# eragonruan/text-detection-ctpn

Hardware: NVIDIA H100
Metric: images/sec @600x900 (higher is better)
Workload: dtype fp32-faithful: fp16 operands + e4m3 cross terms (1 fp16 + 1 e4m3 wgmma per 16 MACs: 2 bf16-rate units per MAC), fp32 accumulate; matmuls around the BiLSTM on bf16x2

## Files before the change

text-detection-ctpn_b200/csrc/common.cuh:

```cuda
#pragma once
#include <cuda_runtime.h>
#include <cuda_bf16.h>
#include <cuda_fp16.h>
#include <stdint.h>
#include <stdio.h>
#include <string.h>

#include "../../include/ctpn_b200.h"

namespace ctpn {

void set_error(const char *fmt, ...);
int cuda_fail(cudaError_t e, const char *what, const char *file, int line);
int current_sm_count(int *sms);

#define CTPN_CUDA(call)                                                        \
  do {                                                                         \
    cudaError_t _e = (call);                                                   \
    if (_e != cudaSuccess) return ::ctpn::cuda_fail(_e, #call, __FILE__, __LINE__); \
  } while (0)

#define CTPN_REQUIRE(cond, ...)                \
  do {                                         \
    if (!(cond)) {                             \
      ::ctpn::set_error(__VA_ARGS__);          \
      return CTPN_ERR_INVALID;                 \
    }                                          \
  } while (0)

#define CTPN_LAUNCH_CHECK()                                                    \
  do {                                                                         \
    cudaError_t _e = cudaGetLastError();                                       \
    if (_e != cudaSuccess) return ::ctpn::cuda_fail(_e, "kernel launch", __FILE__, __LINE__); \
  } while (0)

bool prof_enabled();
struct ProfScope {
  ProfScope(const char *label, double work, cudaStream_t st);
  ~ProfScope();
  cudaStream_t st_;
  int idx_;
};

int conv1_1_tc_ragged(const void *src, int src_is_f32, const float *lut, const float *w_hwio, const float *bias, void *out_planes,
                      int B, int H, int W, int planes, bool outq, float out_s, float out_t, const int *sizes, void *stream);
struct QuantScales { float inv_main, inv_cross, out_s, out_t; };
int conv_tc_run(const void *in_planes, const void *w_planes, const float *bias, void *out, int B, int H, int W, int cin,
                int cout, int taps, int planes, int flags, const QuantScales *q, const int *ext, int ext_shift, void *stream);
int bilstm_ragged(const float *xproj, const float *wh_fw, const float *wh_bw, void *out_planes, int R, int W, int planes,
                  const int *sizes, int rows_per_image, void *stream);

static inline size_t align_up(size_t v, size_t a) { return (v + a - 1) / a * a; }
static inline int ceil_div(int a, int b) { return (a + b - 1) / b; }

__device__ __forceinline__ void split_planes(float a, int planes, __nv_bfloat16 *p) {
  __nv_bfloat16 h0 = __float2bfloat16_rn(a);
  p[0] = h0;
  if (planes > 1) {
    float r1 = __fsub_rn(a, __bfloat162float(h0));
    __nv_bfloat16 h1 = __float2bfloat16_rn(r1);
    p[1] = h1;
    if (planes > 2) {
      float r2 = __fsub_rn(r1, __bfloat162float(h1));
      p[2] = __float2bfloat16_rn(r2);
    }
  }
}

template <int P>
__device__ __forceinline__ void split_planes2(float a, float b, uint32_t (&w)[P]) {
#pragma unroll
  for (int pl = 0; pl < P; ++pl) {
    uint32_t pk;
    asm("cvt.rn.bf16x2.f32 %0, %1, %2;" : "=r"(pk) : "f"(b), "f"(a));
    w[pl] = pk;
    if (pl + 1 < P) {
      a = __fsub_rn(a, __uint_as_float(pk << 16));
      b = __fsub_rn(b, __uint_as_float(pk & 0xffff0000u));
    }
  }
}

constexpr float kResidualGain = 2048.0f;

__device__ __forceinline__ uint32_t f16x2_split(float a, float b, float &ra, float &rb) {
  uint32_t pk;
  asm("cvt.rn.satfinite.f16x2.f32 %0, %1, %2;" : "=r"(pk) : "f"(b), "f"(a));
  const __half2 h = *reinterpret_cast<const __half2 *>(&pk);
  ra = __fsub_rn(a, __low2float(h));
  rb = __fsub_rn(b, __high2float(h));
  return pk;
}
__device__ __forceinline__ uint32_t e4m3x4(float a, float b, float c, float d) {
  uint16_t lo, hi;
  asm("cvt.rn.satfinite.e4m3x2.f32 %0, %1, %2;" : "=h"(lo) : "f"(b), "f"(a));
  asm("cvt.rn.satfinite.e4m3x2.f32 %0, %1, %2;" : "=h"(hi) : "f"(d), "f"(c));
  return (uint32_t)lo | ((uint32_t)hi << 16);
}

__device__ __forceinline__ float2 fmul2_rn(float2 a, float2 b) { return make_float2(__fmul_rn(a.x, b.x), __fmul_rn(a.y, b.y)); }
__device__ __forceinline__ float2 ffma2_rn(float2 a, float2 b, float2 c) {
  return make_float2(__fmaf_rn(a.x, b.x, c.x), __fmaf_rn(a.y, b.y, c.y));
}

__device__ __forceinline__ void f16f8_quad(float v0, float v1, float v2, float v3, float s, float t, float rs, uint32_t &h01,
                                           uint32_t &h23, uint32_t &qv, uint32_t &qr) {
  const float2 a = make_float2(v0, v1), b = make_float2(v2, v3);
  float2 as = a, bs = b;
  if (s != 1.f) {
    as = fmul2_rn(a, make_float2(s, s));
    bs = fmul2_rn(b, make_float2(s, s));
  }
  float2 ra, rb;
  h01 = f16x2_split(as.x, as.y, ra.x, ra.y);
  h23 = f16x2_split(bs.x, bs.y, rb.x, rb.y);
  const float2 at = fmul2_rn(a, make_float2(t, t)), bt = fmul2_rn(b, make_float2(t, t));
  qv = e4m3x4(at.x, at.y, bt.x, bt.y);
  ra = fmul2_rn(ra, make_float2(rs, rs));
  rb = fmul2_rn(rb, make_float2(rs, rs));
  qr = e4m3x4(ra.x, ra.y, rb.x, rb.y);
}

__device__ __forceinline__ uint32_t pack_bf16x2(__nv_bfloat16 lo, __nv_bfloat16 hi) {
  return (uint32_t)__bfloat16_as_ushort(lo) | ((uint32_t)__bfloat16_as_ushort(hi) << 16);
}

__device__ __forceinline__ float bf16_bits_to_float(uint32_t bits16) {
  return __uint_as_float(bits16 << 16);
}

}
```

text-detection-ctpn_b200/csrc/conv1_tc.cu:

```cuda
#include <mutex>

#include "common.cuh"
#include "tc_ptx.cuh"

namespace ctpn {

#ifdef CTPN_DEBUG
#define C1_DBG(p, bit) (((p).debug & (bit)) != 0)
#else
#define C1_DBG(p, bit) false
#endif


constexpr int kC1tThreads = 512;
constexpr int kC1tTileBytes = 128 * 128;
constexpr int kC1tPatch = 3 * 18 * 40;

struct Conv1TcParams {
  const void *src;
  const float *lut, *w, *bias;
  __nv_bfloat16 *out;
  int B, H, W, src_is_f32;
  int tiles_x, tiles_y, total_tiles;
  int debug;
  long long plane_stride;
  float out_s, out_t, out_rs;
  const int *sizes;
};

__device__ __forceinline__ void c1_extent(const Conv1TcParams &p, int b, int &eh, int &ew) {
  eh = p.H; ew = p.W;
  if (p.sizes) {
    eh = min(eh, __ldg(p.sizes + 2 * b));
    ew = min(ew, __ldg(p.sizes + 2 * b + 1));
  }
}

template <int P, int OUTQ>
__global__ void __launch_bounds__(kC1tThreads, 1)
conv1_tc_kernel(const Conv1TcParams p) {
  using namespace ptx;
  extern __shared__ uint8_t smem_raw[];
  const uint32_t raw = smem_u32(smem_raw);
  constexpr int kSPG = P <= 2 ? 2 : 1;
  constexpr int kStages = 2 * kSPG;
  const uint32_t a0 = (raw + 1023u) & ~1023u;
  const uint32_t b0 = a0 + (uint32_t)kStages * P * kC1tTileBytes;
  uint8_t *base = smem_raw + (a0 - raw);
  uint8_t *bsm = base + kStages * P * kC1tTileBytes;
  float *patch = reinterpret_cast<float *>(bsm + P * 64 * 128);
  float *lut_s = patch + 4 * kC1tPatch;
  float *epi = lut_s + 768;
  uint64_t *bars = reinterpret_cast<uint64_t *>(epi + 2 * 128 * 32);
  const uint32_t fullA = smem_u32(bars), emptyA = fullA + 32;

  const int warp = __shfl_sync(0xffffffffu, (int)(threadIdx.x >> 5), 0), lane = threadIdx.x & 31;
  if (threadIdx.x == 0) {
    for (int i = 0; i < 4; ++i) {
      mbar_init(fullA + 8 * i, 128);
      mbar_init(emptyA + 8 * i, 2);
    }
    fence_mbar_init();
  }
  if (!p.src_is_f32)
    for (int i = threadIdx.x; i < 768; i += kC1tThreads) lut_s[i] = p.lut[i];
  for (int i = threadIdx.x; i < 64 * 4; i += kC1tThreads) {
    const int co = i >> 2, chunk = i & 3;
    uint32_t pk[3][4];
#pragma unroll
    for (int j = 0; j < 4; ++j) {
      float v[2];
#pragma unroll
      for (int e = 0; e < 2; ++e) {
        const int k = chunk * 8 + j * 2 + e;
        v[e] = k < 27 ? p.w[k * 64 + co] : (k == 27 ? p.bias[co] : 0.f);
      }
      uint32_t t[P];
      split_planes2<P>(v[0], v[1], t);
#pragma unroll
      for (int pl = 0; pl < P; ++pl) pk[pl][j] = t[pl];
    }
#pragma unroll
    for (int pl = 0; pl < P; ++pl)
      *reinterpret_cast<uint4 *>(bsm + pl * 64 * 128 + co * 128 + ((chunk ^ (co & 7)) << 4)) = make_uint4(pk[pl][0], pk[pl][1], pk[pl][2], pk[pl][3]);
  }
  fence_proxy_async();
  __syncthreads();
  const int tiles_per_img = p.tiles_x * p.tiles_y;

  if (warp < 8) {
    const int grp = warp >> 2;
    const int m = (warp & 3) * 32 + lane, th = m >> 3, tw = m & 7;
    const unsigned tpi = (unsigned)tiles_per_img, tx = (unsigned)p.tiles_x;
    uint32_t raw[2][3];
    unsigned valid = 0;
    auto fetch = [&](int tile) {
      valid = 0;
      if (tile >= p.total_tiles) return;
      const unsigned b = (unsigned)tile / tpi, r = (unsigned)tile % tpi;
      const int y0 = (int)(r / tx) * 16, x0 = (int)(r % tx) * 8;
      int eh, ew;
      c1_extent(p, (int)b, eh, ew);
#pragma unroll
      for (int u = 0; u < 2; ++u) {
        const int i = m + u * 128;
        const int xx = i % 10, yy = i / 10;
        const int gx = x0 + xx - 1, gy = y0 + yy - 1;
        if (i < 180 && gx >= 0 && gx < ew && gy >= 0 && gy < eh && !C1_DBG(p, 1)) {
          const size_t off = (((size_t)b * p.H + gy) * p.W + gx) * 3;
          if (p.src_is_f32) {
            const float *q = reinterpret_cast<const float *>(p.src) + off;
            raw[u][0] = __float_as_uint(q[0]); raw[u][1] = __float_as_uint(q[1]); raw[u][2] = __float_as_uint(q[2]);
          } else {
            const uint8_t *q = reinterpret_cast<const uint8_t *>(p.src) + off;
            raw[u][0] = q[0]; raw[u][1] = q[1]; raw[u][2] = q[2];
          }
          valid |= 1u << u;
        }
      }
    };
    fetch(blockIdx.x + grp * gridDim.x);
    int n = 0;
    for (int tile = blockIdx.x + grp * gridDim.x; tile < p.total_tiles; tile += 2 * gridDim.x, ++n) {
      const int s = grp * kSPG + n % kSPG;
      const uint32_t ph = (uint32_t)(n / kSPG) & 1u;
      float *pt = patch + (grp * 2 + (n & 1)) * kC1tPatch;
#pragma unroll
      for (int u = 0; u < 2; ++u) {
        const int i = m + u * 128;
        if (i < 180) {
          const int xx = i % 10, yy = i / 10;
          float v0 = 0.f, v1 = 0.f, v2 = 0.f;
          if ((valid >> u) & 1u) {
            if (p.src_is_f32) {
              v0 = __uint_as_float(raw[u][0]); v1 = __uint_as_float(raw[u][1]); v2 = __uint_as_float(raw[u][2]);
            } else {
              v0 = lut_s[raw[u][0] * 3 + 0]; v1 = lut_s[raw[u][1] * 3 + 1]; v2 = lut_s[raw[u][2] * 3 + 2];
            }
          }
          pt[(0 * 18 + yy) * 40 + xx] = v0;
          pt[(1 * 18 + yy) * 40 + xx] = v1;
          pt[(2 * 18 + yy) * 40 + xx] = v2;
        }
      }
      fetch(tile + 2 * gridDim.x);
      mbar_wait(emptyA + 8 * s, ph ^ 1u);
      if (grp == 0) asm volatile("bar.sync 1, 128;" ::: "memory");
      else asm volatile("bar.sync 2, 128;" ::: "memory");
      uint8_t *arow = base + s * P * kC1tTileBytes + m * 128;
#pragma unroll
      for (int chunk = 0; chunk < (C1_DBG(p, 2) ? 0 : 4); ++chunk) {
        uint32_t pk[3][4];
#pragma unroll
        for (int j = 0; j < 4; ++j) {
          float v[2];
#pragma unroll
          for (int e = 0; e < 2; ++e) {
            const int k = chunk * 8 + j * 2 + e;
            v[e] = k < 27 ? pt[((k % 3) * 18 + th + k / 9) * 40 + tw + (k / 3) % 3] : (k == 27 ? 1.f : 0.f);
          }
          uint32_t t[P];
          split_planes2<P>(v[0], v[1], t);
#pragma unroll
          for (int pl = 0; pl < P; ++pl) pk[pl][j] = t[pl];
        }
#pragma unroll
        for (int pl = 0; pl < P; ++pl)
          *reinterpret_cast<uint4 *>(arow + pl * kC1tTileBytes + ((chunk ^ (m & 7)) << 4)) = make_uint4(pk[pl][0], pk[pl][1], pk[pl][2], pk[pl][3]);
      }
      fence_proxy_async();
      mbar_arrive(fullA + 8 * s);
    }
  } else {
    const int wg = (warp >> 2) - 2;
    const int cw = warp - 8, chunk = cw >> 2, quarter = cw & 3;
    const int m = quarter * 32 + lane, th = m >> 3, tw = m & 7;
    const int frow = wg * 64 + (warp & 3) * 16 + (lane >> 2);
    constexpr uint32_t kHi = gmma_desc_hi(1024);
    const uint32_t b_lo = gmma_desc_lo(b0);
    float accm[32], accc[32];
    uint4 *stage_w = reinterpret_cast<uint4 *>(epi + chunk * 4096 + quarter * 1024);
    int n = 0;
    for (int tile = blockIdx.x; tile < p.total_tiles; tile += gridDim.x, ++n) {
      const int s = (n & 1) * kSPG + (n >> 1) % kSPG;
      const uint32_t ph = (uint32_t)((n >> 1) / kSPG) & 1u;
      const unsigned b = (unsigned)tile / (unsigned)tiles_per_img, r = (unsigned)tile % (unsigned)tiles_per_img;
      const int y = (int)(r / (unsigned)p.tiles_x) * 16 + th, x = (int)(r % (unsigned)p.tiles_x) * 8 + tw;
      const bool ok = y < p.H && x < p.W;
      int eh, ew;
      c1_extent(p, (int)b, eh, ew);
      const bool live = y < eh && x < ew;
      const long long pix = ((long long)b * p.H + y) * p.W + x;
      const unsigned okmask = __ballot_sync(0xffffffffu, ok);
      long long spix[4];
#pragma unroll
      for (int it = 0; it < 4; ++it) {
        const long long hi = __shfl_sync(0xffffffffu, (int)(pix >> 32), it * 8 + (lane >> 2));
        const unsigned lo = __shfl_sync(0xffffffffu, (unsigned)(pix & 0xffffffffll), it * 8 + (lane >> 2));
        spix[it] = (hi << 32) | lo;
      }
      mbar_wait(fullA + 8 * s, ph);
      const uint32_t a_lo = gmma_desc_lo(a0 + s * P * kC1tTileBytes + wg * 64 * 128);
      wgmma_fence();
#pragma unroll
      for (int i = 0; i < P; ++i)
#pragma unroll
        for (int j = 0; j < P - i; ++j)
#pragma unroll
          for (int k = 0; k < 2; ++k) {
            const uint64_t da = ((uint64_t)kHi << 32) | (a_lo + i * (kC1tTileBytes >> 4) + 2u * k);
            const uint64_t db = ((uint64_t)kHi << 32) | (b_lo + j * ((64 * 128) >> 4) + 2u * k);
            if (i + j == 0) wgmma_bf16(accm, da, db, (uint32_t)k);
            else wgmma_bf16(accc, da, db, (k == 0 && i == 0 && j == 1) ? 0u : 1u);
          }
      wgmma_commit();
      wgmma_wait<0>();
      wgmma_fence_regs(accm);
      if (P > 1) wgmma_fence_regs(accc);
      if ((threadIdx.x & 127) == 0) mbar_arrive(emptyA + 8 * s);
      if (P > 1) {
#pragma unroll
        for (int i = 0; i < 32; ++i) accm[i] = accm[i] + accc[i];
      }
      named_sync(3, 256);
#pragma unroll
      for (int j = 0; j < 8; ++j) {
        const int q = 2 * (j & 3) + ((lane & 3) >> 1);
#pragma unroll
        for (int h = 0; h < 2; ++h) {
          const int row = frow + 8 * h;
          *reinterpret_cast<float2 *>(epi + (j >> 2) * 4096 + row * 32 + ((q ^ (row & 7)) << 2) + 2 * (lane & 1)) =
              make_float2(accm[4 * j + 2 * h], accm[4 * j + 2 * h + 1]);
        }
      }
      named_sync(3, 256);
      if (!C1_DBG(p, 8)) {
        float v[32];
#pragma unroll
        for (int q = 0; q < 8; ++q) {
          const float4 t = *reinterpret_cast<const float4 *>(epi + chunk * 4096 + m * 32 + ((q ^ (m & 7)) << 2));
          v[4 * q + 0] = t.x; v[4 * q + 1] = t.y; v[4 * q + 2] = t.z; v[4 * q + 3] = t.w;
        }
        if (!live) {
#pragma unroll
          for (int i = 0; i < 32; ++i) v[i] = 0.f;
        }
        if (OUTQ) {
          uint32_t wh[16], wq[16];
#pragma unroll
          for (int i = 0; i < 8; ++i) {
            const float v0 = fmaxf(v[4 * i], 0.f), v1 = fmaxf(v[4 * i + 1], 0.f), v2 = fmaxf(v[4 * i + 2], 0.f), v3 = fmaxf(v[4 * i + 3], 0.f);
            f16f8_quad(v0, v1, v2, v3, p.out_s, p.out_t, p.out_rs, wh[2 * i], wh[2 * i + 1], wq[i], wq[8 + i]);
          }
#pragma unroll
          for (int pl = 0; pl < 2; ++pl) {
            __syncwarp();
#pragma unroll
            for (int q = 0; q < 4; ++q) {
              const uint4 val = pl == 0 ? make_uint4(wh[4 * q], wh[4 * q + 1], wh[4 * q + 2], wh[4 * q + 3])
                                        : make_uint4(wq[4 * q], wq[4 * q + 1], wq[4 * q + 2], wq[4 * q + 3]);
              stage_w[lane * 4 + (q ^ ((lane >> 1) & 3))] = val;
            }
            __syncwarp();
            uint8_t *obase = reinterpret_cast<uint8_t *>(p.out) + (long long)pl * p.plane_stride * 2;
            const int j = lane & 3;
            const int off = pl == 0 ? chunk * 64 + j * 16 : chunk * 32 + (j >> 1) * 64 + (j & 1) * 16;
#pragma unroll
            for (int it = 0; it < 4; ++it) {
              const int pp = it * 8 + (lane >> 2);
              const uint4 val = stage_w[pp * 4 + (j ^ ((pp >> 1) & 3))];
              if (((okmask >> pp) & 1u) && !C1_DBG(p, 4)) *reinterpret_cast<uint4 *>(obase + spix[it] * 128 + off) = val;
            }
          }
        } else {
        uint32_t w[P][16];
#pragma unroll
        for (int i = 0; i < 16; ++i) {
          uint32_t t[P];
          split_planes2<P>(fmaxf(v[2 * i], 0.f), fmaxf(v[2 * i + 1], 0.f), t);
#pragma unroll
          for (int pl = 0; pl < P; ++pl) w[pl][i] = t[pl];
        }
#pragma unroll
        for (int pl = 0; pl < P; ++pl) {
          __syncwarp();
#pragma unroll
          for (int q = 0; q < 4; ++q) stage_w[lane * 4 + (q ^ ((lane >> 1) & 3))] = make_uint4(w[pl][4 * q], w[pl][4 * q + 1], w[pl][4 * q + 2], w[pl][4 * q + 3]);
          __syncwarp();
          __nv_bfloat16 *obase = p.out + (long long)pl * p.plane_stride + chunk * 32 + (lane & 3) * 8;
#pragma unroll
          for (int it = 0; it < 4; ++it) {
            const int pp = it * 8 + (lane >> 2);
            const uint4 val = stage_w[pp * 4 + ((lane & 3) ^ ((pp >> 1) & 3))];
            if (((okmask >> pp) & 1u) && !C1_DBG(p, 4)) *reinterpret_cast<uint4 *>(obase + spix[it] * 64) = val;
          }
        }
        }
      }
    }
  }
}

template <int P, int OUTQ = 0>
static int launch_conv1_tc(Conv1TcParams &p, cudaStream_t st) {
  const size_t smem = 1024 + (size_t)(P <= 2 ? 4 : 2) * P * kC1tTileBytes + (size_t)P * 64 * 128 +
                      (4 * kC1tPatch + 768 + 2 * 128 * 32) * sizeof(float) + 64;
  constexpr int kMaxDevices = 64;
  static std::mutex mu;
  static int sm_count[kMaxDevices];
  int dev = 0;
  CTPN_CUDA(cudaGetDevice(&dev));
  CTPN_REQUIRE(dev >= 0 && dev < kMaxDevices, "ctpn_conv1_1_tc: device index %d not supported", dev);
  int sms;
  {
    std::lock_guard<std::mutex> lock(mu);
    if (sm_count[dev] == 0) {
      CTPN_CUDA(cudaFuncSetAttribute(conv1_tc_kernel<P, OUTQ>, cudaFuncAttributeMaxDynamicSharedMemorySize, (int)smem));
      CTPN_CUDA(cudaDeviceGetAttribute(&sm_count[dev], cudaDevAttrMultiProcessorCount, dev));
    }
    sms = sm_count[dev];
  }
  const int grid = p.total_tiles < sms ? p.total_tiles : sms;
  ProfScope prof("conv1_1", 2.0 * p.B * p.H * p.W * 27.0 * 64.0, st);
  conv1_tc_kernel<P, OUTQ><<<grid, kC1tThreads, smem, st>>>(p);
  CTPN_LAUNCH_CHECK();
  return CTPN_OK;
}

}

int ctpn::conv1_1_tc_ragged(const void *src, int src_is_f32, const float *lut, const float *w_hwio, const float *bias,
                            void *out_planes, int B, int H, int W, int planes, bool outq, float out_s, float out_t,
                            const int *sizes, void *stream) {
  CTPN_REQUIRE(src && w_hwio && bias && out_planes, "ctpn_conv1_1_tc: null pointer");
  CTPN_REQUIRE(src_is_f32 || lut, "ctpn_conv1_1_tc: uint8 input needs the mean-subtraction LUT");
  CTPN_REQUIRE(B > 0 && H > 0 && W > 0, "ctpn_conv1_1_tc: bad shape");
  CTPN_REQUIRE(planes >= 1 && planes <= 3, "ctpn_conv1_1_tc: planes must be 1..3");
  Conv1TcParams p;
  p.src = src; p.lut = lut; p.w = w_hwio; p.bias = bias; p.out = (__nv_bfloat16 *)out_planes;
  p.B = B; p.H = H; p.W = W; p.src_is_f32 = src_is_f32;
  p.tiles_x = ceil_div(W, 8); p.tiles_y = ceil_div(H, 16);
  const long long total = (long long)B * p.tiles_x * p.tiles_y;
  CTPN_REQUIRE(total < (1ll << 31), "ctpn_conv1_1_tc: too many tiles");
  p.total_tiles = (int)total;
  p.plane_stride = (long long)B * H * W * 64;
  p.out_s = p.out_t = p.out_rs = 1.f;
  p.sizes = sizes;
  if (outq) {
    CTPN_REQUIRE(out_s > 0.f && out_t > 0.f, "ctpn_conv1_1_tc_f16f8: scales must be positive");
    p.out_s = out_s; p.out_t = out_t; p.out_rs = kResidualGain * out_t / out_s;
  }
#ifdef CTPN_DEBUG
  static const int dbg = [] { const char *e = getenv("CTPN_C1_DEBUG"); return e ? atoi(e) : 0; }();
  p.debug = dbg;
#else
  p.debug = 0;
#endif
  cudaStream_t st = (cudaStream_t)stream;
  if (outq) return launch_conv1_tc<2, 1>(p, st);
  if (planes == 1) return launch_conv1_tc<1>(p, st);
  if (planes == 2) return launch_conv1_tc<2>(p, st);
  return launch_conv1_tc<3>(p, st);
}

using namespace ctpn;

extern "C" int ctpn_conv1_1_tc(const void *src, int src_is_f32, const float *lut, const float *w_hwio, const float *bias,
                               void *out_planes, int B, int H, int W, int planes, void *stream) {
  return conv1_1_tc_ragged(src, src_is_f32, lut, w_hwio, bias, out_planes, B, H, W, planes, false, 1.f, 1.f, nullptr, stream);
}

extern "C" int ctpn_conv1_1_tc_f16f8(const void *src, int src_is_f32, const float *lut, const float *w_hwio, const float *bias,
                                     void *out_planes, int B, int H, int W, float out_s, float out_t, void *stream) {
  return conv1_1_tc_ragged(src, src_is_f32, lut, w_hwio, bias, out_planes, B, H, W, 2, true, out_s, out_t, nullptr, stream);
}
```

text-detection-ctpn_b200/csrc/conv_tc.cu:

```cuda
#include <cuda.h>

#include <algorithm>
#include <mutex>
#include <unordered_map>

#include "common.cuh"
#include "tc_ptx.cuh"
#include "tma_host.cuh"

namespace ctpn {

#ifdef CTPN_DEBUG
#define CTPN_DBG(p, bit) (((p).debug & (bit)) != 0)
#else
#define CTPN_DBG(p, bit) false
#endif

struct ConvTcParams {
  int B, H, W, Cin, Cout, taps, planes, flags;
  int tiles_x, tiles_y, tiles_n, total_tiles;
  int m_tiles, total_units;
  int TH, TW, tw_log2;
  int PW;
  int patch_bytes;
  int patch_tx_bytes;
  int group_stride_bytes;
  int cout_pad;
  int Ho, Wo;
  int stages_a, stages_b;
  int debug;
  const float *bias;
  void *out;
  long long out_plane_stride;
  float inv_main, inv_cross, out_s, out_t, out_rs;
  int in_stack_h, out_rows, out_stacked;
  const int *ext;
  int ext_shift, ext_n;
  double work;
  int promote_every;
};

template <int BN, int PR> constexpr bool kEpiWarpgroup = !PR && BN <= 128;
template <int BN, int PR> constexpr int kTcThreads = kEpiWarpgroup<BN, PR> ? 512 : 384;
constexpr int kMaxStages = 8;
constexpr int kCtrlBytes = 8 * (4 * kMaxStages) + 16;
constexpr int kEpiBytes = 2 * 128 * 32 * 4;
constexpr int kXposeBytes = 4 * 512;

struct EpiPixel {
  bool ok, live;
  int oy, ox;
  long long pix;
  unsigned okmask;
  long long spix[4];
};

__device__ __forceinline__ void epi_pixel(const ConvTcParams &p, int mt, int m, int lane, EpiPixel &e) {
  const int th = m >> p.tw_log2, tw = m & (p.TW - 1);
  const int tiles_per_img = p.tiles_x * p.tiles_y;
  const int b = mt / tiles_per_img, r = mt % tiles_per_img;
  const int y = (r / p.tiles_x) * p.TH + th, x = (r % p.tiles_x) * p.TW + tw;
  e.live = true;
  int ob = b;
  if (p.flags & CTPN_F_POOL) {
    e.oy = y >> 1; e.ox = x >> 1;
    e.ok = !(th & 1) && !(tw & 1) && e.oy < p.Ho && e.ox < p.Wo;
  } else {
    e.oy = y; e.ox = x;
    e.ok = y < p.H && x < p.W;
    if (p.in_stack_h) {
      ob = y / p.in_stack_h;
      e.oy = y - ob * p.in_stack_h;
      e.live = e.oy < p.in_stack_h - 1;
      if (!p.out_stacked) e.ok = e.ok && e.live;
    }
  }
  if (p.ext) {
    const int ib = min(ob, p.ext_n - 1);
    e.live = e.live && e.oy < (__ldg(p.ext + 2 * ib) >> p.ext_shift) && e.ox < (__ldg(p.ext + 2 * ib + 1) >> p.ext_shift);
  }
  e.pix = ((long long)ob * p.out_rows + e.oy) * p.Wo + e.ox;
  e.okmask = __ballot_sync(0xffffffffu, e.ok);
#pragma unroll
  for (int it = 0; it < 4; ++it) {
    const long long hi = __shfl_sync(0xffffffffu, (int)(e.pix >> 32), it * 8 + (lane >> 2));
    const unsigned lo = __shfl_sync(0xffffffffu, (unsigned)(e.pix & 0xffffffffll), it * 8 + (lane >> 2));
    e.spix[it] = (hi << 32) | lo;
  }
}

__device__ __forceinline__ void store_transposed(uint4 *stage_w, const uint32_t (&w)[16], uint8_t *obase, long long row_bytes,
                                                 const EpiPixel &e, bool st_ok, bool small, int lane) {
  const int j = lane & 3;
  if (!small) {
    __syncwarp();
#pragma unroll
    for (int q = 0; q < 4; ++q) stage_w[lane * 4 + (q ^ ((lane >> 1) & 3))] = make_uint4(w[4 * q], w[4 * q + 1], w[4 * q + 2], w[4 * q + 3]);
    __syncwarp();
    if (st_ok) {
#pragma unroll
      for (int it = 0; it < 4; ++it) {
        const int pp = it * 8 + (lane >> 2);
        const uint4 val = stage_w[pp * 4 + (j ^ ((pp >> 1) & 3))];
        if ((e.okmask >> pp) & 1u) *reinterpret_cast<uint4 *>(obase + e.spix[it] * row_bytes) = val;
      }
    }
  } else {
#pragma unroll
    for (int it = 0; it < 4; ++it) {
      __syncwarp();
      if ((lane >> 3) == it) {
        const int row = lane & 7;
#pragma unroll
        for (int q = 0; q < 4; ++q) stage_w[row * 4 + (q ^ ((row >> 1) & 3))] = make_uint4(w[4 * q], w[4 * q + 1], w[4 * q + 2], w[4 * q + 3]);
      }
      __syncwarp();
      const int row = lane >> 2, pp = it * 8 + row;
      const uint4 val = stage_w[row * 4 + (j ^ ((row >> 1) & 3))];
      if (st_ok && ((e.okmask >> pp) & 1u)) *reinterpret_cast<uint4 *>(obase + e.spix[it] * row_bytes) = val;
    }
  }
}

template <int P, int F8>
__device__ __forceinline__ void epi_chunk(const ConvTcParams &p, const EpiPixel &e, float (&v)[32], int c0, uint4 *stage_w,
                                          bool small, bool bias_relu, int lane) {
  const bool pool = (p.flags & CTPN_F_POOL) != 0, relu = (p.flags & CTPN_F_RELU) != 0;
  const bool out_f32 = (p.flags & CTPN_F_OUT_F32) != 0;
  if (bias_relu) {
#pragma unroll
    for (int q = 0; q < 8; ++q) {
      const float4 bq = __ldg(reinterpret_cast<const float4 *>(p.bias + c0) + q);
      v[4 * q + 0] += bq.x;
      v[4 * q + 1] += bq.y;
      v[4 * q + 2] += bq.z;
      v[4 * q + 3] += bq.w;
    }
    if (relu) {
#pragma unroll
      for (int i = 0; i < 32; ++i) v[i] = fmaxf(v[i], 0.f);
    }
  }
  if (!e.live) {
#pragma unroll
    for (int i = 0; i < 32; ++i) v[i] = 0.f;
  }
  if (pool) {
#pragma unroll
    for (int i = 0; i < 32; ++i) {
      v[i] = fmaxf(v[i], __shfl_xor_sync(0xffffffffu, v[i], 1));
      v[i] = fmaxf(v[i], __shfl_xor_sync(0xffffffffu, v[i], p.TW));
    }
  }
  if (F8 && pool && !out_f32 && !(p.flags & CTPN_F_OUT_BF16X2)) {
    const int j = (lane & 1) | ((lane >> 2) & 2);
    float x[8];
#pragma unroll
    for (int k = 0; k < 8; ++k) x[k] = j == 0 ? v[k] : j == 1 ? v[8 + k] : j == 2 ? v[16 + k] : v[24 + k];
    const bool okw = e.oy < p.Ho && e.ox < p.Wo;
    uint4 hw;
    uint2 qv, qr;
    f16f8_quad(x[0], x[1], x[2], x[3], p.out_s, p.out_t, p.out_rs, hw.x, hw.y, qv.x, qr.x);
    f16f8_quad(x[4], x[5], x[6], x[7], p.out_s, p.out_t, p.out_rs, hw.z, hw.w, qv.y, qr.y);
    if (okw && c0 < p.Cout && !CTPN_DBG(p, 8)) {
      uint8_t *o0 = reinterpret_cast<uint8_t *>(p.out) + e.pix * p.Cout * 2;
      uint8_t *o1 = o0 + p.out_plane_stride * 2 + (long long)(c0 >> 6) * 128 + (c0 & 63) + j * 8;
      *reinterpret_cast<uint4 *>(o0 + (long long)c0 * 2 + j * 16) = hw;
      *reinterpret_cast<uint2 *>(o1) = qv;
      *reinterpret_cast<uint2 *>(o1 + 64) = qr;
    }
  } else if (F8 && !out_f32 && !(p.flags & CTPN_F_OUT_BF16X2)) {
    uint32_t wh[16], wq[16];
#pragma unroll
    for (int i = 0; i < 8; ++i) {
      f16f8_quad(v[4 * i], v[4 * i + 1], v[4 * i + 2], v[4 * i + 3], p.out_s, p.out_t, p.out_rs, wh[2 * i], wh[2 * i + 1], wq[i], wq[8 + i]);
    }
    const int j = lane & 3;
    const bool st_ok = c0 < p.Cout && !CTPN_DBG(p, 8);
    uint8_t *obase = reinterpret_cast<uint8_t *>(p.out);
    store_transposed(stage_w, wh, obase + (long long)c0 * 2 + j * 16, (long long)p.Cout * 2, e, st_ok, small, lane);
    store_transposed(stage_w, wq, obase + p.out_plane_stride * 2 + (long long)(c0 >> 6) * 128 + (c0 & 63) + (j >> 1) * 64 + (j & 1) * 16,
                     (long long)p.Cout * 2, e, st_ok, small, lane);
  } else if (!out_f32) {
    uint32_t w[P][16];
#pragma unroll
    for (int i = 0; i < 16; ++i) {
      uint32_t t[P];
      split_planes2<P>(v[2 * i], v[2 * i + 1], t);
#pragma unroll
      for (int pl = 0; pl < P; ++pl) w[pl][i] = t[pl];
    }
#pragma unroll
    for (int pl = 0; pl < P; ++pl) {
      uint8_t *obase = reinterpret_cast<uint8_t *>(reinterpret_cast<__nv_bfloat16 *>(p.out) + (long long)pl * p.out_plane_stride + c0 + (lane & 3) * 8);
      store_transposed(stage_w, w[pl], obase, (long long)p.Cout * 2, e, c0 < p.Cout && !CTPN_DBG(p, 8), small, lane);
    }
  } else if (e.ok && c0 < p.Cout && !CTPN_DBG(p, 8)) {
    float4 *dst = reinterpret_cast<float4 *>(reinterpret_cast<float *>(p.out) + e.pix * p.Cout + c0);
#pragma unroll
    for (int q = 0; q < 8; ++q) dst[q] = make_float4(v[4 * q], v[4 * q + 1], v[4 * q + 2], v[4 * q + 3]);
  }
}

template <int BN, int P, int TAPS, int MC, int F8, int PR = 0>
__global__ void __launch_bounds__(kTcThreads<BN, PR>, 1)
conv_tc_kernel(const __grid_constant__ CUtensorMap tmap_a, const __grid_constant__ CUtensorMap tmap_b,
               const ConvTcParams p) {
  using namespace ptx;
  constexpr int kBBytes = BN * 128;
  constexpr bool EW = kEpiWarpgroup<BN, PR>;
  static_assert(!F8 || P == 2, "F16F8 uses two stage slots per operand");
  static_assert(!PR || (P == 3 && !F8), "promotion is built for three bf16 planes");
  extern __shared__ uint8_t smem_raw[];
  const uint32_t raw = smem_u32(smem_raw);
  const uint32_t ring_a = (raw + 1023u) & ~1023u;
  const uint32_t a_stage = (uint32_t)P * p.patch_bytes, b_stage = (uint32_t)P * kBBytes;
  const uint32_t ring_b = ring_a + (uint32_t)p.stages_a * a_stage;
  float *epi = reinterpret_cast<float *>(smem_raw + (ring_b - raw) + (size_t)p.stages_b * b_stage);
  uint4 *xpose = reinterpret_cast<uint4 *>(reinterpret_cast<uint8_t *>(epi) + kEpiBytes);
  uint8_t *ctrl = reinterpret_cast<uint8_t *>(epi) + kEpiBytes + (EW ? kXposeBytes : 0);
  const uint32_t fullA = smem_u32(ctrl), emptyA = fullA + 8 * kMaxStages;
  const uint32_t fullB = emptyA + 8 * kMaxStages, emptyB = fullB + 8 * kMaxStages;
  const uint32_t epiF = emptyB + 8 * kMaxStages, epiE = epiF + 8;

  const int warp = __shfl_sync(0xffffffffu, (int)(threadIdx.x >> 5), 0), lane = threadIdx.x & 31;
  if (threadIdx.x == 0) {
    prefetch_tmap(&tmap_a);
    prefetch_tmap(&tmap_b);
    for (int s = 0; s < kMaxStages; ++s) {
      mbar_init(fullA + 8 * s, 1);
      mbar_init(emptyA + 8 * s, 2);
      mbar_init(fullB + 8 * s, 1);
      mbar_init(emptyB + 8 * s, MC ? 4 : 2);
    }
    mbar_init(epiF, 256);
    mbar_init(epiE, 128);
    fence_mbar_init();
  }
  __syncthreads();
  if (MC) cluster_sync_all();
  const uint32_t rank = MC ? cluster_ctarank() : 0u;
  const int u_begin = MC ? (int)(blockIdx.x >> 1) : (int)blockIdx.x, u_step = MC ? (int)(gridDim.x >> 1) : (int)gridDim.x;
  auto unit_tile = [&](int u, int &mt, int &nt) {
    nt = u % p.tiles_n;
    mt = u / p.tiles_n;
    if (MC) mt = min(2 * mt + (int)rank, p.m_tiles - 1);
  };

  const int kblocks = p.Cin / 64;
  const int tiles_per_img = p.tiles_x * p.tiles_y;
  constexpr int halo = TAPS == 9 ? 1 : 0;

  if (warp < 4) {
    if (EW) regs_dealloc<24>();
    else regs_dealloc<40>();
    if (warp == 1) {
      int s = 0;
      uint32_t ph = 0;
      for (int u = u_begin; u < p.total_units; u += u_step) {
        int mt, nt;
        unit_tile(u, mt, nt);
        const int b = mt / tiles_per_img, r = mt % tiles_per_img;
        const int y0 = (r / p.tiles_x) * p.TH - halo, x0 = (r % p.tiles_x) * p.TW - halo;
        for (int kb = 0; kb < kblocks; ++kb) {
          mbar_wait(emptyA + 8 * s, ph ^ 1u);
          if (elect_one()) {
            if (CTPN_DBG(p, 2)) { mbar_arrive(fullA + 8 * s); }
            else {
              mbar_arrive_expect_tx(fullA + 8 * s, (uint32_t)P * (uint32_t)p.patch_tx_bytes);
              for (int pl = 0; pl < P; ++pl)
                tma_load_4d(&tmap_a, fullA + 8 * s, ring_a + s * a_stage + pl * p.patch_bytes, kb * 64, x0, y0, pl * p.B + b);
            }
          }
          __syncwarp();
          if (++s == p.stages_a) { s = 0; ph ^= 1u; }
        }
      }
    } else if (warp == 0) {
      int s = 0;
      uint32_t ph = 0;
      for (int u = u_begin; u < p.total_units; u += u_step) {
        int mt, nt;
        unit_tile(u, mt, nt);
        for (int kb = 0; kb < kblocks; ++kb) {
          for (int tap = 0; tap < TAPS; ++tap) {
            mbar_wait(emptyB + 8 * s, ph ^ 1u);
            if (elect_one()) {
              if (CTPN_DBG(p, 1)) { mbar_arrive(fullB + 8 * s); }
              else {
                mbar_arrive_expect_tx(fullB + 8 * s, b_stage);
                for (int pl = 0; pl < P; ++pl) {
                  if (MC)
                    tma_load_2d_mc(&tmap_b, fullB + 8 * s, ring_b + s * b_stage + pl * kBBytes + rank * (kBBytes / 2),
                                   tap * p.Cin + kb * 64, pl * p.cout_pad + nt * BN + (int)rank * (BN / 2), (uint16_t)3);
                  else
                    tma_load_2d(&tmap_b, fullB + 8 * s, ring_b + s * b_stage + pl * kBBytes, tap * p.Cin + kb * 64,
                                pl * p.cout_pad + nt * BN);
                }
              }
            }
            __syncwarp();
            if (++s == p.stages_b) { s = 0; ph ^= 1u; }
          }
        }
      }
    }
  } else if (EW && warp >= 12) {
    regs_alloc<152>();
    const int m = (warp & 3) * 32 + lane;
    uint4 *stage_w = xpose + (warp & 3) * 32;
    uint32_t eph = 0;
    if (!CTPN_DBG(p, 16)) {
      for (int u = u_begin; u < p.total_units; u += u_step) {
        int mt, nt;
        unit_tile(u, mt, nt);
        EpiPixel e;
        epi_pixel(p, mt, m, lane, e);
#pragma unroll 1
        for (int c2 = 0; c2 < BN / 64; ++c2) {
          float v[2][32];
          mbar_wait(epiF, eph);
#pragma unroll
          for (int es = 0; es < 2; ++es) {
#pragma unroll
            for (int q = 0; q < 8; ++q) {
              const float4 t = *reinterpret_cast<const float4 *>(epi + es * 4096 + m * 32 + ((q ^ (m & 7)) << 2));
              v[es][4 * q + 0] = t.x; v[es][4 * q + 1] = t.y; v[es][4 * q + 2] = t.z; v[es][4 * q + 3] = t.w;
            }
          }
          mbar_arrive(epiE);
          eph ^= 1u;
#pragma unroll
          for (int es = 0; es < 2; ++es) epi_chunk<P, F8>(p, e, v[es], nt * BN + (2 * c2 + es) * 32, stage_w, true, false, lane);
        }
      }
    }
  } else {
    if (EW) regs_alloc<168>();
    else regs_alloc<232>();
    const int wg = (warp >> 2) - 1;
    const bool leader = (threadIdx.x & 127) == 0;
    constexpr int R = BN / 2;
    float accm[R], accc[R];
    float accs[R];
#ifdef CTPN_DEBUG
    const int pe = PR ? p.promote_every : 1;
#else
    constexpr int pe = 1;
#endif
    constexpr uint32_t kPatch16 = (TAPS == 9 ? 23552u : 16384u) >> 4;
    constexpr uint32_t kB16 = (uint32_t)kBBytes >> 4;
    constexpr uint32_t kHiB = gmma_desc_hi(1024);
    const uint32_t hi_a = gmma_desc_hi((uint32_t)p.group_stride_bytes);
    const uint32_t wg_off = (uint32_t)wg * 8u * (uint32_t)p.group_stride_bytes;
    int sa = 0, sb = 0, prev_b = -1, prev_a = -1;
    uint32_t pha = 0, phb = 0, eph = 0;
    const int frow = wg * 64 + (warp & 3) * 16 + (lane >> 2);
    auto stage_half = [&](int c2) {
#pragma unroll
      for (int j = 0; j < 8; ++j) {
        const int i8 = c2 * 8 + j, q = 2 * (j & 3) + ((lane & 3) >> 1);
#pragma unroll
        for (int h = 0; h < 2; ++h) {
          const int row = frow + 8 * h;
          *reinterpret_cast<float2 *>(epi + (j >> 2) * 4096 + row * 32 + ((q ^ (row & 7)) << 2) + 2 * (lane & 1)) =
              make_float2(accm[4 * i8 + 2 * h], accm[4 * i8 + 2 * h + 1]);
        }
      }
    };
    auto release = [&](int sbx, int sax) {
      if (leader) {
        if (MC) {
          mbar_arrive_cluster(emptyB + 8 * sbx, 0u);
          mbar_arrive_cluster(emptyB + 8 * sbx, 1u);
        } else {
          mbar_arrive(emptyB + 8 * sbx);
        }
        if (sax >= 0) mbar_arrive(emptyA + 8 * sax);
      }
    };
    for (int u = u_begin; u < p.total_units; u += u_step) {
      if (PR) {
#pragma unroll
        for (int i = 0; i < R; ++i) accs[i] = 0.f;
      }
      for (int kb = 0; kb < kblocks; ++kb) {
        if (p.stages_a == 1 && prev_a >= 0) {
          wgmma_wait<0>();
          release(prev_b, prev_a);
          prev_b = prev_a = -1;
        }
        mbar_wait(fullA + 8 * sa, pha);
        const uint32_t a_lo = gmma_desc_lo(ring_a + sa * a_stage + wg_off);
#pragma unroll
        for (int tap = 0; tap < TAPS; ++tap) {
          mbar_wait(fullB + 8 * sb, phb);
          const uint32_t b_lo = gmma_desc_lo(ring_b + sb * b_stage);
          constexpr int kPW = 10;
          const uint32_t view16 = TAPS == 9 ? (uint32_t)((tap / 3) * kPW + tap % 3) * 8u : 0u;
          const uint32_t not_first = (kb | tap) != 0;
          const int step = kb * TAPS + tap;
          wgmma_fence();
          if (!CTPN_DBG(p, 4)) {
            if (F8) {
#pragma unroll
              for (int k = 0; k < 4; ++k)
                wgmma_f16(accm, ((uint64_t)hi_a << 32) | (a_lo + view16 + 2u * k), ((uint64_t)kHiB << 32) | (b_lo + 2u * k),
                          k == 0 ? not_first : 1u);
#pragma unroll
              for (int k = 0; k < 4; ++k)
                wgmma_e4m3(accc, ((uint64_t)hi_a << 32) | (a_lo + kPatch16 + view16 + 2u * k),
                           ((uint64_t)kHiB << 32) | (b_lo + kB16 + 2u * k), k == 0 ? not_first : 1u);
            } else if (PR) {
              const uint32_t chain_on = step % pe != 0;
#pragma unroll
              for (int k = 0; k < 4; ++k)
                wgmma_bf16(accm, ((uint64_t)hi_a << 32) | (a_lo + view16 + 2u * k), ((uint64_t)kHiB << 32) | (b_lo + 2u * k),
                           k == 0 ? chain_on : 1u);
              wgmma_commit();
#pragma unroll
              for (int i = 0; i < P; ++i) {
#pragma unroll
                for (int j = (i == 0); j < P - i; ++j) {
#pragma unroll
                  for (int k = 0; k < 4; ++k) {
                    const uint64_t da = ((uint64_t)hi_a << 32) | (a_lo + i * kPatch16 + view16 + 2u * k);
                    const uint64_t db = ((uint64_t)kHiB << 32) | (b_lo + j * kB16 + 2u * k);
                    wgmma_bf16(accc, da, db, (k == 0 && i == 0 && j == 1) ? not_first : 1u);
                  }
                }
              }
            } else {
#pragma unroll
              for (int i = 0; i < P; ++i) {
#pragma unroll
                for (int j = 0; j < P - i; ++j) {
#pragma unroll
                  for (int k = 0; k < 4; ++k) {
                    const uint64_t da = ((uint64_t)hi_a << 32) | (a_lo + i * kPatch16 + view16 + 2u * k);
                    const uint64_t db = ((uint64_t)kHiB << 32) | (b_lo + j * kB16 + 2u * k);
                    if (i + j == 0) wgmma_bf16(accm, da, db, k == 0 ? not_first : 1u);
                    else wgmma_bf16(accc, da, db, (k == 0 && i == 0 && j == 1) ? not_first : 1u);
                  }
                }
              }
            }
          }
          wgmma_commit();
          wgmma_wait<1>();
          if (prev_b >= 0) release(prev_b, prev_a);
          prev_b = sb;
          prev_a = tap == TAPS - 1 ? sa : -1;
          if (PR && ((step + 1) % pe == 0 || step == kblocks * TAPS - 1)) {
            wgmma_fence_regs(accm);
#pragma unroll
            for (int i = 0; i < R; ++i) accs[i] = __fadd_rn(accs[i], accm[i]);
          }
          if (++sb == p.stages_b) { sb = 0; phb ^= 1u; }
        }
        if (++sa == p.stages_a) { sa = 0; pha ^= 1u; }
      }
      wgmma_wait<0>();
      wgmma_fence_regs(accm);
      if (P > 1) wgmma_fence_regs(accc);
      if (prev_b >= 0) release(prev_b, prev_a);
      prev_b = prev_a = -1;
      if (P > 1) {
#pragma unroll
        for (int i = 0; i < R; ++i)
          accm[i] = F8 ? __fmaf_rn(accc[i], p.inv_cross, accm[i] * p.inv_main) : PR ? __fadd_rn(accs[i], accc[i]) : accm[i] + accc[i];
      }

      if (CTPN_DBG(p, 16)) continue;
      if (EW) {
        const float *bt = p.bias + (u % p.tiles_n) * BN + 2 * (lane & 3);
#pragma unroll
        for (int i8 = 0; i8 < BN / 8; ++i8) {
          const float2 bq = __ldg(reinterpret_cast<const float2 *>(bt + 8 * i8));
#pragma unroll
          for (int h = 0; h < 2; ++h) {
            accm[4 * i8 + 2 * h] += bq.x;
            accm[4 * i8 + 2 * h + 1] += bq.y;
          }
        }
        if (p.flags & CTPN_F_RELU) {
#pragma unroll
          for (int i = 0; i < R; ++i) accm[i] = fmaxf(accm[i], 0.f);
        }
#pragma unroll
        for (int c2 = 0; c2 < BN / 64; ++c2) {
          mbar_wait(epiE, eph ^ 1u);
          stage_half(c2);
          mbar_arrive(epiF);
          eph ^= 1u;
        }
      } else {
        const int cw = warp - 4, eset = cw >> 2, quarter = cw & 3;
        const int m = quarter * 32 + lane;
        int mt, nt;
        unit_tile(u, mt, nt);
        EpiPixel e;
        epi_pixel(p, mt, m, lane, e);
        uint4 *stage_w = reinterpret_cast<uint4 *>(epi + eset * 4096 + quarter * 1024);
#pragma unroll
        for (int c2 = 0; c2 < BN / 64; ++c2) {
          named_sync(1, 256);
          stage_half(c2);
          named_sync(1, 256);
          float v[32];
#pragma unroll
          for (int q = 0; q < 8; ++q) {
            const float4 t = *reinterpret_cast<const float4 *>(epi + eset * 4096 + m * 32 + ((q ^ (m & 7)) << 2));
            v[4 * q + 0] = t.x; v[4 * q + 1] = t.y; v[4 * q + 2] = t.z; v[4 * q + 3] = t.w;
          }
          epi_chunk<P, F8>(p, e, v, nt * BN + (2 * c2 + eset) * 32, stage_w, false, true, lane);
        }
      }
    }
  }
  __syncthreads();
  if (MC) cluster_sync_all();
}


constexpr int kMaxDevices = 64;
static std::mutex g_mu;
static int g_sms[kMaxDevices];

struct Tuning { int debug = 0, bn = 0, stages_a = 0, stages_b = 0, mcast = 1, promote = 1; };
static const Tuning &tuning() {
  static const Tuning t = [] {
    Tuning v;
#ifdef CTPN_DEBUG
    auto env_int = [](const char *name, int dflt) { const char *e = getenv(name); return e ? atoi(e) : dflt; };
    v.debug = env_int("CTPN_TC_DEBUG", 0);
    v.bn = env_int("CTPN_TC_BN", 0);
    v.stages_a = env_int("CTPN_TC_STAGES_A", 0);
    v.stages_b = env_int("CTPN_TC_STAGES_B", 0);
    v.mcast = env_int("CTPN_TC_MCAST", 1);
    v.promote = std::max(1, env_int("CTPN_TC_PROMOTE", 1));
#endif
    return v;
  }();
  return t;
}

struct TmapKey {
  const void *ptr;
  unsigned long long d0, d1, d2, d3;
  unsigned b0, b1, b2, b3;
  int dev;
  bool operator==(const TmapKey &o) const {
    return ptr == o.ptr && d0 == o.d0 && d1 == o.d1 && d2 == o.d2 && d3 == o.d3 && b0 == o.b0 && b1 == o.b1 && b2 == o.b2 &&
           b3 == o.b3 && dev == o.dev;
  }
};
struct TmapKeyHash {
  size_t operator()(const TmapKey &k) const {
    size_t h = std::hash<const void *>()(k.ptr);
    for (unsigned long long v : {k.d0, k.d1, k.d2, k.d3, (unsigned long long)k.b0, (unsigned long long)k.b1,
                                 (unsigned long long)k.b2, (unsigned long long)k.b3, (unsigned long long)k.dev})
      h = h * 1000003u ^ std::hash<unsigned long long>()(v);
    return h;
  }
};
static std::unordered_map<TmapKey, CUtensorMap, TmapKeyHash> g_tmaps;

static int cached_tmap(int dev, CUtensorMap *out, const void *ptr, int rank, const cuuint64_t *dims, const cuuint64_t *strides,
                       const cuuint32_t *box) {
  TmapKey k{ptr, dims[0], dims[1], rank > 2 ? dims[2] : 0, rank > 3 ? dims[3] : 0, box[0], box[1], rank > 2 ? box[2] : 0,
            rank > 3 ? box[3] : 0, dev};
  std::lock_guard<std::mutex> lock(g_mu);
  auto it = g_tmaps.find(k);
  if (it != g_tmaps.end()) { *out = it->second; return CTPN_OK; }
  EncodeTiledFn enc = nullptr;
  int rc = tma_get_encode(&enc);
  if (rc) return rc;
  if ((rc = tma_encode_bf16(enc, out, const_cast<void *>(ptr), rank, dims, strides, box))) return rc;
  if (g_tmaps.size() >= 1024) g_tmaps.clear();
  g_tmaps.emplace(k, *out);
  return CTPN_OK;
}

template <int BN, int P, int TAPS, int MC, int F8 = 0, int PR = 0>
static int launch_bn(int dev, const CUtensorMap &ta, const CUtensorMap &tb, ConvTcParams &p, cudaStream_t st) {
  const size_t a_stage = (size_t)p.planes * p.patch_bytes, b_stage = (size_t)p.planes * BN * 128;
  const size_t epi_bytes = kEpiBytes + (kEpiWarpgroup<BN, PR> ? kXposeBytes : 0);
  const size_t budget = 227 * 1024 - 1024 - kCtrlBytes - epi_bytes;
  int sa = (2 * a_stage + 2 * b_stage <= budget) ? 2 : 1;
  if (p.taps == 1) sa = (int)std::min<size_t>(4, std::max<size_t>(1, (budget / 2) / a_stage));
  CTPN_REQUIRE(sa * a_stage + 2 * b_stage <= budget, "conv_tc: pipeline stages (%zu + 2 x %zu B) do not fit in shared memory", a_stage, b_stage);
  int sb = (int)((budget - sa * a_stage) / b_stage);
  if (sb > kMaxStages) sb = kMaxStages;
  if (tuning().stages_a > 0) sa = std::max(1, std::min(sa, tuning().stages_a));
  if (tuning().stages_b > 0) sb = std::max(2, std::min(sb, tuning().stages_b));
  p.stages_a = sa;
  p.stages_b = sb;
  const size_t smem = 1024 + sa * a_stage + sb * b_stage + epi_bytes + kCtrlBytes;
  CTPN_REQUIRE(smem <= 227 * 1024, "conv_tc: %zu bytes of shared memory", smem);
  auto kernel = conv_tc_kernel<BN, P, TAPS, MC, F8, PR>;
  static bool attr_set[kMaxDevices];
  static int max_clusters[kMaxDevices];
  cudaLaunchConfig_t cfg = {};
  cudaLaunchAttribute attr;
  attr.id = cudaLaunchAttributeClusterDimension;
  attr.val.clusterDim.x = 2; attr.val.clusterDim.y = 1; attr.val.clusterDim.z = 1;
  cfg.blockDim = dim3(kTcThreads<BN, PR>);
  cfg.dynamicSmemBytes = smem;
  cfg.stream = st;
  cfg.attrs = &attr;
  cfg.numAttrs = MC ? 1 : 0;
  {
    std::lock_guard<std::mutex> lock(g_mu);
    if (!attr_set[dev]) {
      CTPN_CUDA(cudaFuncSetAttribute(kernel, cudaFuncAttributeMaxDynamicSharedMemorySize, 227 * 1024));
      if (MC) {
        cfg.gridDim = dim3(2 * (g_sms[dev] / 2));
        int n = 0;
        CTPN_CUDA(cudaOccupancyMaxActiveClusters(&n, kernel, &cfg));
        CTPN_REQUIRE(n > 0, "conv_tc: no 2-CTA cluster of this kernel fits on the device");
        max_clusters[dev] = n;
      }
      attr_set[dev] = true;
    }
  }
  char label[128];
  if (prof_enabled()) snprintf(label, sizeof(label), "conv_tc t%d %dx%dx%d c%d-%d %s%d bn%d%s%s", p.taps, p.B, p.H, p.W, p.Cin, p.Cout, F8 ? "f16f8 p" : "p", p.planes, BN, MC ? " mc" : "", PR ? " promote" : "");
  ProfScope prof(label, p.work, st);
  if (MC) cfg.gridDim = dim3(2 * std::min(max_clusters[dev], p.total_units));
  else cfg.gridDim = dim3(std::min(p.total_units, g_sms[dev]));
  CTPN_CUDA(cudaLaunchKernelEx(&cfg, kernel, ta, tb, p));
  CTPN_LAUNCH_CHECK();
  return CTPN_OK;
}

int conv_tc_run(const void *in_planes, const void *w_planes, const float *bias, void *out, int B, int H, int W, int cin,
                int cout, int taps, int planes, int flags, const QuantScales *q, const int *ext, int ext_shift, void *stream) {
  const bool f8 = q != nullptr, promote = (flags & CTPN_F_PROMOTE) != 0;
  CTPN_REQUIRE(f8 || !(flags & CTPN_F_OUT_BF16X2), "ctpn_conv3x3: CTPN_F_OUT_BF16X2 is a flag of ctpn_conv3x3_f16f8");
  CTPN_REQUIRE(!(promote && f8), "ctpn_conv3x3_f16f8: CTPN_F_PROMOTE is a flag of ctpn_conv3x3 with planes = 3");
  CTPN_REQUIRE(!promote || planes == 3, "ctpn_conv3x3: CTPN_F_PROMOTE needs planes = 3 (got %d)", planes);
  CTPN_REQUIRE(in_planes && w_planes && bias && out, "ctpn_conv3x3: null pointer");
  CTPN_REQUIRE(taps == 9 || taps == 1, "ctpn_conv3x3: taps must be 9 or 1 (got %d)", taps);
  CTPN_REQUIRE(planes >= 1 && planes <= 3, "ctpn_conv3x3: planes must be 1..3 (got %d)", planes);
  CTPN_REQUIRE(cin % 64 == 0 && cin >= 64, "ctpn_conv3x3: Cin must be a multiple of 64 (got %d)", cin);
  CTPN_REQUIRE(cout % 64 == 0 && cout >= 64, "ctpn_conv3x3: Cout must be a multiple of 64 (got %d)", cout);
  CTPN_REQUIRE(B > 0 && H > 0 && W > 0, "ctpn_conv3x3: bad shape");
  const bool pool = flags & CTPN_F_POOL;
  CTPN_REQUIRE(!pool || (taps == 9 && H >= 2 && W >= 2), "ctpn_conv3x3: pooling needs taps=9 and H,W >= 2");
  const bool stack_in = flags & CTPN_F_STACK_IN, stack_out = flags & CTPN_F_STACK_OUT;
  CTPN_REQUIRE(!stack_in || (taps == 9 && !pool), "ctpn_conv3x3: CTPN_F_STACK_IN needs taps=9 and no pooling");
  CTPN_REQUIRE(!stack_out || !(flags & CTPN_F_OUT_F32), "ctpn_conv3x3: stacked output is a plane format");
  const int img_B = B, img_H = H;
  if (stack_in) {
    CTPN_REQUIRE((long long)B * (H + 1) < (1ll << 30), "ctpn_conv3x3: stack too tall");
    H = B * (H + 1);
    B = 1;
  }
  int dev = 0, rc;
  CTPN_CUDA(cudaGetDevice(&dev));
  CTPN_REQUIRE(dev >= 0 && dev < kMaxDevices, "ctpn_conv3x3: device index %d not supported", dev);
  {
    std::lock_guard<std::mutex> lock(g_mu);
    if (g_sms[dev] == 0) CTPN_CUDA(cudaDeviceGetAttribute(&g_sms[dev], cudaDevAttrMultiProcessorCount, dev));
  }

  ConvTcParams p;
  memset(&p, 0, sizeof(p));
  p.B = B; p.H = H; p.W = W; p.Cin = cin; p.Cout = cout; p.taps = taps; p.planes = planes; p.flags = flags;
  if (taps == 9) {
    p.TH = 16; p.TW = 8; p.tw_log2 = 3;
    p.PW = 10;
    p.group_stride_bytes = p.PW * 128;
    p.patch_tx_bytes = p.PW * 18 * 128;
    p.patch_bytes = (int)align_up((size_t)p.patch_tx_bytes, 1024);
  } else {
    p.TH = 1; p.TW = 128; p.tw_log2 = 7;
    p.PW = 128;
    p.group_stride_bytes = 1024;
    p.patch_tx_bytes = 128 * 128;
    p.patch_bytes = 128 * 128;
  }
  p.tiles_x = ceil_div(W, p.TW);
  p.tiles_y = ceil_div(H, p.TH);
  p.Ho = pool ? H / 2 : H;
  p.Wo = pool ? W / 2 : W;
  p.bias = bias;
  p.out = out;
  p.work = 2.0 * img_B * img_H * W * (double)taps * cin * cout;
  p.in_stack_h = stack_in ? img_H + 1 : 0;
  const int img_Ho = pool ? img_H / 2 : img_H;
  p.out_rows = img_Ho + (stack_out ? 1 : 0);
  p.out_stacked = stack_out ? 1 : 0;
  p.out_plane_stride = (long long)img_B * p.out_rows * p.Wo * cout;
  p.cout_pad = cout;
  p.ext = ext;
  p.ext_shift = ext_shift;
  p.ext_n = img_B;
  if (f8) {
    CTPN_REQUIRE(q->inv_main > 0.f && q->inv_cross > 0.f && q->out_s > 0.f && q->out_t > 0.f, "ctpn_conv3x3_f16f8: scales must be positive");
    p.inv_main = q->inv_main; p.inv_cross = q->inv_cross; p.out_s = q->out_s; p.out_t = q->out_t;
    p.out_rs = kResidualGain * q->out_t / q->out_s;
  }
  p.debug = tuning().debug;
  p.promote_every = tuning().promote;

  int BN = tuning().bn > 0 ? tuning().bn : (planes == 1 ? 256 : 128);
  if (!(BN == 64 || BN == 128 || BN == 256)) BN = 256;
  if (planes > 1 && BN > 128) BN = 128;
  while (BN > cout || cout % BN) BN >>= 1;
  const long long m_tiles = (long long)B * p.tiles_x * p.tiles_y;
  constexpr long long kMcMaxTilesPerSm = 16;
  const bool mc = taps == 9 && tuning().mcast != 0 && m_tiles >= 2 &&
                  (promote || m_tiles * (cout / BN) < kMcMaxTilesPerSm * g_sms[dev]);
  if (promote && taps == 9 && !mc && BN > 64) BN = 64;
  p.tiles_n = cout / BN;
  const long long total = m_tiles * p.tiles_n;
  CTPN_REQUIRE(total < (1ll << 31), "ctpn_conv3x3: too many tiles");
  p.total_tiles = (int)total;
  p.m_tiles = (int)m_tiles;
  p.total_units = mc ? (int)((m_tiles + 1) / 2) * p.tiles_n : p.total_tiles;

  CUtensorMap ta, tb;
  {
    const int halo = taps == 9 ? 1 : 0;
    cuuint64_t dims[4] = {(cuuint64_t)cin, (cuuint64_t)W, (cuuint64_t)H, (cuuint64_t)planes * B};
    cuuint64_t strides[3] = {(cuuint64_t)cin * 2, (cuuint64_t)W * cin * 2, (cuuint64_t)H * W * cin * 2};
    cuuint32_t box[4] = {64, (cuuint32_t)p.PW, (cuuint32_t)(p.TH + 2 * halo), 1};
    if ((rc = cached_tmap(dev, &ta, in_planes, 4, dims, strides, box))) return rc;
  }
  {
    cuuint64_t dims[2] = {(cuuint64_t)taps * cin, (cuuint64_t)planes * cout};
    cuuint64_t strides[1] = {(cuuint64_t)taps * cin * 2};
    cuuint32_t box[2] = {64, (cuuint32_t)(mc ? BN / 2 : BN)};
    if ((rc = cached_tmap(dev, &tb, w_planes, 2, dims, strides, box))) return rc;
  }
  cudaStream_t st = (cudaStream_t)stream;
#define CTPN_TC_CASE(BN_, P_, T_) \
  if (BN == BN_ && planes == P_ && taps == T_) return launch_bn<BN_, P_, T_, 0>(dev, ta, tb, p, st)
#define CTPN_TC_CASE_MC(BN_, P_) \
  if (mc && BN == BN_ && planes == P_) return launch_bn<BN_, P_, 9, 1>(dev, ta, tb, p, st)
  if (f8) {
    if (mc && BN == 128) return launch_bn<128, 2, 9, 1, 1>(dev, ta, tb, p, st);
    if (mc && BN == 64) return launch_bn<64, 2, 9, 1, 1>(dev, ta, tb, p, st);
    if (taps == 9 && BN == 128) return launch_bn<128, 2, 9, 0, 1>(dev, ta, tb, p, st);
    if (taps == 9 && BN == 64) return launch_bn<64, 2, 9, 0, 1>(dev, ta, tb, p, st);
    if (taps == 1 && BN == 128) return launch_bn<128, 2, 1, 0, 1>(dev, ta, tb, p, st);
    if (taps == 1 && BN == 64) return launch_bn<64, 2, 1, 0, 1>(dev, ta, tb, p, st);
    set_error("ctpn_conv3x3_f16f8: no kernel for BN=%d taps=%d", BN, taps);
    return CTPN_ERR_INVALID;
  }
  if (promote) {
    if (mc && BN == 128) return launch_bn<128, 3, 9, 1, 0, 1>(dev, ta, tb, p, st);
    if (mc && BN == 64) return launch_bn<64, 3, 9, 1, 0, 1>(dev, ta, tb, p, st);
    if (taps == 9 && BN == 64) return launch_bn<64, 3, 9, 0, 0, 1>(dev, ta, tb, p, st);
    if (taps == 1 && BN == 128) return launch_bn<128, 3, 1, 0, 0, 1>(dev, ta, tb, p, st);
    if (taps == 1 && BN == 64) return launch_bn<64, 3, 1, 0, 0, 1>(dev, ta, tb, p, st);
    set_error("ctpn_conv3x3: no promoted kernel for BN=%d taps=%d", BN, taps);
    return CTPN_ERR_INVALID;
  }
  CTPN_TC_CASE_MC(256, 1); CTPN_TC_CASE_MC(128, 1); CTPN_TC_CASE_MC(64, 1);
  CTPN_TC_CASE_MC(128, 2); CTPN_TC_CASE_MC(64, 2);
  CTPN_TC_CASE_MC(128, 3); CTPN_TC_CASE_MC(64, 3);
  CTPN_TC_CASE(256, 1, 9); CTPN_TC_CASE(128, 1, 9); CTPN_TC_CASE(64, 1, 9);
  CTPN_TC_CASE(128, 2, 9); CTPN_TC_CASE(64, 2, 9);
  CTPN_TC_CASE(128, 3, 9); CTPN_TC_CASE(64, 3, 9);
  CTPN_TC_CASE(256, 1, 1); CTPN_TC_CASE(128, 1, 1); CTPN_TC_CASE(64, 1, 1);
  CTPN_TC_CASE(128, 2, 1); CTPN_TC_CASE(64, 2, 1);
  CTPN_TC_CASE(128, 3, 1); CTPN_TC_CASE(64, 3, 1);
#undef CTPN_TC_CASE_MC
#undef CTPN_TC_CASE
  set_error("ctpn_conv3x3: no kernel for BN=%d planes=%d taps=%d", BN, planes, taps);
  return CTPN_ERR_INVALID;
}

}

using namespace ctpn;

extern "C" int ctpn_conv3x3(const void *in_planes, const void *w_planes, const float *bias, void *out, int B, int H,
                            int W, int cin, int cout, int taps, int planes, int flags, void *stream) {
  return conv_tc_run(in_planes, w_planes, bias, out, B, H, W, cin, cout, taps, planes, flags, nullptr, nullptr, 0, stream);
}

extern "C" int ctpn_conv3x3_f16f8(const void *in_planes, const void *w_planes, const float *bias, void *out, int B, int H,
                                  int W, int cin, int cout, int taps, int flags, float inv_main, float inv_cross, float out_s,
                                  float out_t, void *stream) {
  const QuantScales q{inv_main, inv_cross, out_s, out_t};
  return conv_tc_run(in_planes, w_planes, bias, out, B, H, W, cin, cout, taps, 2, flags, &q, nullptr, 0, stream);
}
```

text-detection-ctpn_b200/csrc/net.cu:

```cuda
#include <algorithm>
#include <map>
#include <string>
#include <vector>

#include <cuda_fp8.h>

#include <cmath>

#include "common.cuh"
#ifdef CTPN_DEBUG
#include "testing/ctpn_b200_testing.h"
#endif

namespace ctpn {

struct ConvSpec { const char *name; int cin, cout; bool pool; };
static const ConvSpec kConvs[14] = {
    {"conv1_1", 3, 64, false},    {"conv1_2", 64, 64, true},    {"conv2_1", 64, 128, false},
    {"conv2_2", 128, 128, true},  {"conv3_1", 128, 256, false}, {"conv3_2", 256, 256, false},
    {"conv3_3", 256, 256, true},  {"conv4_1", 256, 512, false}, {"conv4_2", 512, 512, false},
    {"conv4_3", 512, 512, true},  {"conv5_1", 512, 512, false}, {"conv5_2", 512, 512, false},
    {"conv5_3", 512, 512, false}, {"rpn_conv/3x3", 512, 512, false}};
static const char *kFw = "lstm_o/bidirectional_rnn/fw/lstm_cell";
static const char *kBw = "lstm_o/bidirectional_rnn/bw/lstm_cell";
static const double kPixelMeans[3] = {102.9801, 115.9465, 122.7717};

struct Tap { const void *ptr; long long pixels; int channels; bool planes; float q_s = 0.f, q_t = 0.f; int stack_h = 0, stack_w = 0; };

}

using namespace ctpn;

struct ctpn_net {
  int planes = 2;
  bool f16f8 = false, calibrated = false;
  bool promote = false;
  float w_s[14] = {0}, w_t[14] = {0}, act_s[14] = {0}, act_t[14] = {0}, act_max[14] = {0};
  unsigned *absmax_dev = nullptr;
  int conv_simt = 0, keep = 0;
  std::map<std::string, std::vector<float>> host;
  bool dirty = true;
  std::vector<void *> owned;
  float *c11_w = nullptr, *c11_b = nullptr, *lut = nullptr;
  void *conv_w[14] = {nullptr};
  float *conv_b[14] = {nullptr};
  void *xproj_w = nullptr, *fc_w = nullptr, *head_w = nullptr;
  float *xproj_b = nullptr, *fc_b = nullptr, *head_b = nullptr, *wh_fw = nullptr, *wh_bw = nullptr;
  std::map<std::string, Tap> taps;
};

namespace ctpn {

static int dev_alloc(ctpn_net *n, void **p, size_t bytes) {
  CTPN_CUDA(cudaMalloc(p, bytes));
  n->owned.push_back(*p);
  return CTPN_OK;
}

static int upload(ctpn_net *n, float **dst, const float *src, size_t count) {
  int rc = dev_alloc(n, (void **)dst, count * sizeof(float));
  if (rc) return rc;
  CTPN_CUDA(cudaMemcpy(*dst, src, count * sizeof(float), cudaMemcpyHostToDevice));
  return CTPN_OK;
}

static int upload_packed(ctpn_net *n, void **dst, const float *src, int taps, int cin, int cout, int cout_pad) {
  float *tmp = nullptr;
  const size_t cnt = (size_t)taps * cin * cout;
  CTPN_CUDA(cudaMalloc(&tmp, cnt * sizeof(float)));
  cudaError_t e = cudaMemcpy(tmp, src, cnt * sizeof(float), cudaMemcpyHostToDevice);
  int rc = e == cudaSuccess ? dev_alloc(n, dst, (size_t)n->planes * cout_pad * taps * cin * 2) : cuda_fail(e, "memcpy", __FILE__, __LINE__);
  if (!rc) rc = ctpn_pack_weights(tmp, taps, cin, cout, cout_pad, n->planes, *dst, nullptr);
  if (!rc) { e = cudaDeviceSynchronize(); if (e != cudaSuccess) rc = cuda_fail(e, "sync", __FILE__, __LINE__); }
  cudaFree(tmp);
  return rc;
}

static int upload_packed_f16f8(ctpn_net *n, void **dst, const float *src, int cin, int cout, float *s_w, float *t_w) {
  const size_t cnt = (size_t)9 * cin * cout;
  float mx = 0.f;
  for (size_t i = 0; i < cnt; ++i) mx = std::max(mx, fabsf(src[i]));
  if (!(mx > 0.f) || !std::isfinite(mx)) { set_error("weights are all zero or not finite"); return CTPN_ERR_INVALID; }
  *s_w = exp2f(floorf(log2f(16384.f / mx)));
  *t_w = exp2f(floorf(log2f(448.f / mx)));
  float *tmp = nullptr;
  CTPN_CUDA(cudaMalloc(&tmp, cnt * sizeof(float)));
  cudaError_t e = cudaMemcpy(tmp, src, cnt * sizeof(float), cudaMemcpyHostToDevice);
  int rc = e == cudaSuccess ? dev_alloc(n, dst, (size_t)2 * cout * 9 * cin * 2) : cuda_fail(e, "memcpy", __FILE__, __LINE__);
  if (!rc) rc = ctpn_pack_weights_f16f8(tmp, 9, cin, cout, cout, *s_w, *t_w, *dst, nullptr);
  if (!rc) { e = cudaDeviceSynchronize(); if (e != cudaSuccess) rc = cuda_fail(e, "sync", __FILE__, __LINE__); }
  cudaFree(tmp);
  return rc;
}

static void free_device(ctpn_net *n) {
  for (void *p : n->owned) cudaFree(p);
  n->owned.clear();
  n->absmax_dev = nullptr;
  n->calibrated = false;
}

static const std::vector<float> *need(ctpn_net *n, const std::string &name, size_t count) {
  auto it = n->host.find(name);
  if (it == n->host.end()) { set_error("weight '%s' has not been set", name.c_str()); return nullptr; }
  if (it->second.size() != count) {
    set_error("weight '%s' has %zu elements, expected %zu", name.c_str(), it->second.size(), count);
    return nullptr;
  }
  return &it->second;
}

static int finalize(ctpn_net *n) {
  if (!n->dirty) return CTPN_OK;
  free_device(n);
  int rc;
  {
    std::vector<float> lut(256 * 3);
    for (int v = 0; v < 256; ++v)
      for (int c = 0; c < 3; ++c) lut[v * 3 + c] = (float)((double)v - kPixelMeans[c]);
    if ((rc = upload(n, &n->lut, lut.data(), lut.size()))) return rc;
  }
  for (int l = 0; l < 14; ++l) {
    const ConvSpec &s = kConvs[l];
    const auto *w = need(n, std::string(s.name) + "/weights", (size_t)9 * s.cin * s.cout);
    const auto *b = need(n, std::string(s.name) + "/biases", s.cout);
    if (!w || !b) return CTPN_ERR_INVALID;
    if (l == 0) {
      if ((rc = upload(n, &n->c11_w, w->data(), w->size()))) return rc;
      if ((rc = upload(n, &n->c11_b, b->data(), b->size()))) return rc;
    } else {
      if (n->f16f8) rc = upload_packed_f16f8(n, &n->conv_w[l], w->data(), s.cin, s.cout, &n->w_s[l], &n->w_t[l]);
      else rc = upload_packed(n, &n->conv_w[l], w->data(), 9, s.cin, s.cout, s.cout);
      if (rc) return rc;
      if ((rc = upload(n, &n->conv_b[l], b->data(), b->size()))) return rc;
    }
  }
  {
    const auto *kf = need(n, std::string(kFw) + "/kernel", 640 * 512), *kb = need(n, std::string(kBw) + "/kernel", 640 * 512);
    const auto *bf = need(n, std::string(kFw) + "/bias", 512), *bb = need(n, std::string(kBw) + "/bias", 512);
    if (!kf || !kb || !bf || !bb) return CTPN_ERR_INVALID;
    std::vector<float> wx((size_t)512 * 1024), bx(1024);
    for (int k = 0; k < 512; ++k)
      for (int c = 0; c < 512; ++c) {
        wx[(size_t)k * 1024 + c] = (*kf)[(size_t)k * 512 + c];
        wx[(size_t)k * 1024 + 512 + c] = (*kb)[(size_t)k * 512 + c];
      }
    for (int c = 0; c < 512; ++c) { bx[c] = (*bf)[c]; bx[512 + c] = (*bb)[c]; }
    if ((rc = upload_packed(n, &n->xproj_w, wx.data(), 1, 512, 1024, 1024))) return rc;
    if ((rc = upload(n, &n->xproj_b, bx.data(), bx.size()))) return rc;
    if ((rc = upload(n, &n->wh_fw, kf->data() + 512 * 512, 128 * 512))) return rc;
    if ((rc = upload(n, &n->wh_bw, kb->data() + 512 * 512, 128 * 512))) return rc;
  }
  {
    const auto *w = need(n, "lstm_o/weights", 256 * 512), *b = need(n, "lstm_o/biases", 512);
    if (!w || !b) return CTPN_ERR_INVALID;
    if ((rc = upload_packed(n, &n->fc_w, w->data(), 1, 256, 512, 512))) return rc;
    if ((rc = upload(n, &n->fc_b, b->data(), b->size()))) return rc;
  }
  {
    const auto *wb = need(n, "rpn_bbox_pred/weights", 512 * 40), *bb = need(n, "rpn_bbox_pred/biases", 40);
    const auto *wc = need(n, "rpn_cls_score/weights", 512 * 20), *bc = need(n, "rpn_cls_score/biases", 20);
    if (!wb || !bb || !wc || !bc) return CTPN_ERR_INVALID;
    std::vector<float> w((size_t)512 * 64, 0.f), b(64, 0.f);
    for (int k = 0; k < 512; ++k) {
      for (int c = 0; c < 40; ++c) w[(size_t)k * 64 + c] = (*wb)[(size_t)k * 40 + c];
      for (int c = 0; c < 20; ++c) w[(size_t)k * 64 + 40 + c] = (*wc)[(size_t)k * 20 + c];
    }
    for (int c = 0; c < 40; ++c) b[c] = (*bb)[c];
    for (int c = 0; c < 20; ++c) b[40 + c] = (*bc)[c];
    if ((rc = upload_packed(n, &n->head_w, w.data(), 1, 512, 64, 64))) return rc;
    if ((rc = upload(n, &n->head_b, b.data(), b.size()))) return rc;
  }
  if (n->f16f8 && (rc = dev_alloc(n, (void **)&n->absmax_dev, sizeof(unsigned)))) return rc;
  n->dirty = false;
  return CTPN_OK;
}

struct ConvLayer {
  size_t in, out;
  int h, w, ho, wo;
  int flags;
  int shift;
  bool stacked;
  long long elems;
};

struct NetLayout {
  bool stack;
  ConvLayer conv[14];
  size_t lstm, fc, xproj, heads, total;
  int fh, fw;
};

static NetLayout net_layout(const ctpn_net *n, int B, int H, int W) {
  NetLayout L;
  const int P = n->planes;
  int h = H, w = W, shift = 0;
  for (int l = 0; l < 14; ++l) {
    ConvLayer &c = L.conv[l];
    c.h = h; c.w = w;
    if (kConvs[l].pool) { h /= 2; w /= 2; ++shift; }
    c.ho = h; c.wo = w; c.shift = shift;
  }
  L.fh = h; L.fw = w;
  L.stack = !n->conv_simt && ((long long)B * (h + 1) + 15) / 16 < (long long)B * ((h + 15) / 16);
  size_t sizes[16];
  for (int l = 0; l < 14; ++l) {
    const ConvSpec &s = kConvs[l];
    ConvLayer &c = L.conv[l];
    c.stacked = L.stack && l >= 9 && l <= 12;
    c.flags = 0;
    if (l > 0) {
      c.flags = CTPN_F_RELU | (s.pool ? CTPN_F_POOL : 0) | (n->promote ? CTPN_F_PROMOTE : 0);
      if (n->f16f8 && l == 13) c.flags |= CTPN_F_OUT_BF16X2;
      if (c.stacked) c.flags |= CTPN_F_STACK_OUT;
      if (L.stack && l >= 10) c.flags |= CTPN_F_STACK_IN;
    }
    c.elems = (long long)B * (c.ho + (c.stacked ? 1 : 0)) * c.wo * s.cout;
    sizes[l] = (size_t)P * c.elems * 2;
  }
  const size_t M = (size_t)B * h * w;
  sizes[14] = (size_t)P * M * 256 * 2;
  sizes[15] = (size_t)P * M * 512 * 2;
  size_t act[16], o = 0;
  if (n->keep) {
    for (int i = 0; i < 16; ++i) { act[i] = o; o = align_up(o + sizes[i], 1024); }
  } else {
    size_t even = 0, odd = 0;
    for (int i = 0; i < 16; ++i) (i & 1 ? odd : even) = std::max(i & 1 ? odd : even, sizes[i]);
    even = align_up(even, 1024); odd = align_up(odd, 1024);
    for (int i = 0; i < 16; ++i) act[i] = (i & 1) ? even : 0;
    o = even + odd;
  }
  for (int l = 0; l < 14; ++l) { L.conv[l].in = l ? act[l - 1] : 0; L.conv[l].out = act[l]; }
  L.lstm = act[14]; L.fc = act[15];
  L.xproj = o; o = align_up(o + M * 1024 * sizeof(float), 1024);
  L.heads = o; o = align_up(o + M * 64 * sizeof(float), 1024);
  L.total = o;
  return L;
}

__global__ void split_heads_kernel(const float *__restrict__ heads, long long M, float *__restrict__ cls, float *__restrict__ bbox) {
  const long long i = (long long)blockIdx.x * blockDim.x + threadIdx.x;
  if (i >= M * 64) return;
  const long long m = i >> 6;
  const int c = (int)(i & 63);
  const float v = heads[i];
  if (c < 40) bbox[m * 40 + c] = v;
  else if (c < 60) cls[m * 20 + (c - 40)] = v;
}

__global__ void f16f8_to_f32_kernel(const __half *__restrict__ hi, const uint8_t *__restrict__ cross, long long n, int C, float s, float t,
                                    int stack_h, int stack_w, float *__restrict__ dst) {
  const long long i = (long long)blockIdx.x * blockDim.x + threadIdx.x;
  if (i >= n) return;
  long long pix = i / C;
  const int c = (int)(i % C);
  if (stack_h) {
    const long long per = (long long)stack_h * stack_w, b = pix / per, r = pix % per;
    pix = b * (stack_h + 1) * stack_w + r;
  }
  const uint8_t rb = cross[pix * 2 * C + (c >> 6) * 128 + 64 + (c & 63)];
  const __half_raw hr = __nv_cvt_fp8_to_halfraw((__nv_fp8_storage_t)rb, __NV_E4M3);
  const float r = __half2float(__half(hr)) / (kResidualGain * t / s);
  dst[i] = (__half2float(hi[pix * C + c]) + r) / s;
}

__global__ void planes_to_f32_kernel(const __nv_bfloat16 *__restrict__ src, long long n, long long plane_stride, int planes, int C,
                                     int stack_h, int stack_w, float *__restrict__ dst) {
  const long long i = (long long)blockIdx.x * blockDim.x + threadIdx.x;
  if (i >= n) return;
  long long j = i;
  if (stack_h) {
    const long long pix = i / C, per = (long long)stack_h * stack_w;
    j = ((pix / per) * (stack_h + 1) * stack_w + pix % per) * C + i % C;
  }
  float v = __bfloat162float(src[j]);
  if (planes > 1) v += __bfloat162float(src[j + plane_stride]);
  if (planes > 2) v += __bfloat162float(src[j + 2 * plane_stride]);
  dst[i] = v;
}

__global__ void absmax_f16_kernel(const __half *__restrict__ x, long long n, unsigned *__restrict__ out) {
  float m = 0.f;
  for (long long i = (long long)blockIdx.x * blockDim.x + threadIdx.x; i < n; i += (long long)gridDim.x * blockDim.x)
    m = fmaxf(m, fabsf(__half2float(x[i])));
  unsigned bits = __float_as_uint(m);
  if (m != m) bits = 0x7fc00000u;
  for (int o = 16; o; o >>= 1) bits = max(bits, __shfl_xor_sync(0xffffffffu, bits, o));
  if ((threadIdx.x & 31) == 0) atomicMax(out, bits);
}

static int run_conv(ctpn_net *n, const NetLayout &L, int l, const void *images, int src_is_f32, const int *sizes, int B,
                    char *ws, float out_s, float out_t, void *stream) {
  const ConvSpec &s = kConvs[l];
  const ConvLayer &c = L.conv[l];
  if (!n->f16f8 || (c.flags & CTPN_F_OUT_BF16X2)) out_s = out_t = 1.f;
  if (c.stacked && !(c.flags & CTPN_F_STACK_IN))
    CTPN_CUDA(cudaMemsetAsync(ws + c.out, 0, (size_t)n->planes * c.elems * 2, (cudaStream_t)stream));
#ifdef CTPN_DEBUG
  if (n->conv_simt)
    return l == 0 ? ctpn_conv1_1(images, src_is_f32, n->lut, n->c11_w, n->c11_b, ws + c.out, B, c.h, c.w, n->planes, stream)
                  : ctpn_conv3x3_simt(ws + c.in, n->conv_w[l], n->conv_b[l], ws + c.out, B, c.h, c.w, s.cin, s.cout, 9, n->planes,
                                      c.flags, stream);
#endif
  if (l == 0)
    return conv1_1_tc_ragged(images, src_is_f32, n->lut, n->c11_w, n->c11_b, ws + c.out, B, c.h, c.w, n->planes, n->f16f8, out_s,
                             out_t, sizes, stream);
  QuantScales q{};
  if (n->f16f8) q = {1.f / (n->act_s[l - 1] * n->w_s[l]), 1.f / (kResidualGain * n->act_t[l - 1] * n->w_t[l]), out_s, out_t};
  return conv_tc_run(ws + c.in, n->conv_w[l], n->conv_b[l], ws + c.out, B, c.h, c.w, s.cin, s.cout, 9, n->planes, c.flags,
                     n->f16f8 ? &q : nullptr, sizes, c.shift, stream);
}

static int calibrate_f16f8(ctpn_net *n, const void *images, int src_is_f32, const int *sizes, int B, const NetLayout &L, char *ws,
                           void *stream) {
  cudaStream_t st = (cudaStream_t)stream;
  for (int l = 0; l < 13; ++l) {
    const ConvLayer &c = L.conv[l];
    float s_try = 1.f;
    for (int attempt = 0; ; ++attempt) {
      int rc = run_conv(n, L, l, images, src_is_f32, sizes, B, ws, s_try, 1.f, stream);
      if (rc) return rc;
      CTPN_CUDA(cudaMemsetAsync(n->absmax_dev, 0, sizeof(unsigned), st));
      absmax_f16_kernel<<<1184, 256, 0, st>>>((const __half *)(ws + c.out), c.elems, n->absmax_dev);
      CTPN_LAUNCH_CHECK();
      unsigned bits = 0;
      CTPN_CUDA(cudaMemcpyAsync(&bits, n->absmax_dev, sizeof(unsigned), cudaMemcpyDeviceToHost, st));
      CTPN_CUDA(cudaStreamSynchronize(st));
      float mx;
      memcpy(&mx, &bits, sizeof(float));
      CTPN_REQUIRE(mx == mx, "calibration: layer %s produced NaN", kConvs[l].name);
      if (std::isinf(mx) || mx >= 60000.f) {
        CTPN_REQUIRE(attempt < 6, "calibration: activations of %s exceed 65504 * 2^48", kConvs[l].name);
        s_try *= 1.f / 256.f;
        continue;
      }
      const float amax = std::max(mx / s_try, 1e-20f);
      n->act_max[l] = amax;
      n->act_s[l] = amax * s_try > 16384.f || s_try < 1.f ? exp2f(floorf(log2f(16384.f / amax))) : 1.f;
      n->act_t[l] = exp2f(floorf(log2f(448.f / amax)) - 2.f);
      break;
    }
    int rc = run_conv(n, L, l, images, src_is_f32, sizes, B, ws, n->act_s[l], n->act_t[l], stream);
    if (rc) return rc;
  }
  n->calibrated = true;
  return CTPN_OK;
}

}

extern "C" int ctpn_net_create(ctpn_net_t **net, int planes) {
  CTPN_REQUIRE(net, "ctpn_net_create: null pointer");
  CTPN_REQUIRE((planes >= 1 && planes <= 3) || planes == CTPN_ARITH_F16F8 || planes == CTPN_ARITH_BF16X3P,
               "ctpn_net_create: planes must be 1..3, CTPN_ARITH_F16F8 or CTPN_ARITH_BF16X3P (got %d)", planes);
  ctpn_net *n = new ctpn_net();
  n->f16f8 = planes == CTPN_ARITH_F16F8;
  n->promote = planes == CTPN_ARITH_BF16X3P;
  n->planes = n->f16f8 ? 2 : n->promote ? 3 : planes;
  *net = n;
  return CTPN_OK;
}

extern "C" int ctpn_net_destroy(ctpn_net_t *net) {
  if (!net) return CTPN_OK;
  free_device(net);
  delete net;
  return CTPN_OK;
}

extern "C" int ctpn_net_set_option(ctpn_net_t *net, const char *key, int value) {
  CTPN_REQUIRE(net && key, "ctpn_net_set_option: null pointer");
  if (!strcmp(key, "keep_activations")) net->keep = value != 0;
  else if (!strcmp(key, "recalibrate")) net->calibrated = false;
#ifdef CTPN_DEBUG
  else if (!strcmp(key, "conv_simt")) {
    CTPN_REQUIRE(!value || !net->f16f8, "ctpn_net_set_option: the SIMT reference kernels read bf16 planes, not F16F8");
    net->conv_simt = value != 0;
  }
#endif
  else { set_error("ctpn_net_set_option: unknown key '%s'", key); return CTPN_ERR_INVALID; }
  return CTPN_OK;
}

extern "C" int ctpn_net_set_weight(ctpn_net_t *net, const char *name, const float *data_host, size_t count) {
  CTPN_REQUIRE(net && name && data_host, "ctpn_net_set_weight: null pointer");
  net->host[name].assign(data_host, data_host + count);
  net->dirty = true;
  return CTPN_OK;
}

extern "C" int ctpn_net_feature_hw(int H, int W, int *fh, int *fw) {
  CTPN_REQUIRE(fh && fw && H >= 16 && W >= 16, "ctpn_net_feature_hw: image must be at least 16x16");
  *fh = H / 2 / 2 / 2 / 2;
  *fw = W / 2 / 2 / 2 / 2;
  return CTPN_OK;
}

extern "C" size_t ctpn_net_workspace_bytes(const ctpn_net_t *net, int B, int H, int W) {
  if (!net || B <= 0 || H < 16 || W < 16) return 0;
  return net_layout(net, B, H, W).total;
}

static int net_forward(ctpn_net *net, const void *images, int src_is_f32, const int *sizes, int B, int H, int W,
                       float *cls_score_out, float *bbox_pred_out, void *workspace, size_t workspace_bytes, void *stream) {
#ifdef CTPN_DEBUG
  CTPN_REQUIRE(!sizes || !net->conv_simt, "ctpn_net_forward_ragged: the SIMT reference kernels take uniform batches only");
#endif
  int rc = finalize(net);
  if (rc) return rc;
  const NetLayout L = net_layout(net, B, H, W);
  if (workspace_bytes < L.total) {
    set_error("ctpn_net_forward: workspace %zu < %zu bytes", workspace_bytes, L.total);
    return CTPN_ERR_WORKSPACE;
  }
  char *ws = (char *)workspace;
  const int P = net->planes;
  net->taps.clear();
  if (net->f16f8 && !net->calibrated && (rc = calibrate_f16f8(net, images, src_is_f32, sizes, B, L, ws, stream))) return rc;
  for (int l = 0; l < 14; ++l) {
    const ConvSpec &s = kConvs[l];
    const ConvLayer &c = L.conv[l];
    if ((rc = run_conv(net, L, l, images, src_is_f32, sizes, B, ws, net->act_s[l], net->act_t[l], stream))) return rc;
    const bool q = net->f16f8 && !(c.flags & CTPN_F_OUT_BF16X2);
    net->taps[s.pool ? std::string(s.name) + "+pool" : std::string(s.name)] =
        Tap{ws + c.out, (long long)B * c.ho * c.wo, s.cout, true, q ? net->act_s[l] : 0.f, q ? net->act_t[l] : 0.f,
            c.stacked ? c.ho : 0, c.stacked ? c.wo : 0};
  }
  const int M = B * L.fh * L.fw;
  const int pf = net->promote ? CTPN_F_PROMOTE : 0;
  auto gemm = [&](const void *in, const void *w, const float *b, void *out, int cin, int cout, int flags) {
#ifdef CTPN_DEBUG
    if (net->conv_simt) return ctpn_conv3x3_simt(in, w, b, out, 1, 1, M, cin, cout, 1, P, flags, stream);
#endif
    return conv_tc_run(in, w, b, out, 1, 1, M, cin, cout, 1, P, flags, nullptr, nullptr, 0, stream);
  };
  if ((rc = gemm(ws + L.conv[13].out, net->xproj_w, net->xproj_b, ws + L.xproj, 512, 1024, CTPN_F_OUT_F32 | pf))) return rc;
  net->taps["xproj"] = Tap{ws + L.xproj, M, 1024, false};
  if ((rc = bilstm_ragged((const float *)(ws + L.xproj), net->wh_fw, net->wh_bw, ws + L.lstm, B * L.fh, L.fw, P, sizes, L.fh, stream))) return rc;
  net->taps["lstm_out"] = Tap{ws + L.lstm, M, 256, true};
  if ((rc = gemm(ws + L.lstm, net->fc_w, net->fc_b, ws + L.fc, 256, 512, pf))) return rc;
  net->taps["lstm_o"] = Tap{ws + L.fc, M, 512, true};
  if ((rc = gemm(ws + L.fc, net->head_w, net->head_b, ws + L.heads, 512, 64, CTPN_F_OUT_F32 | pf))) return rc;
  const long long tot = (long long)M * 64;
  split_heads_kernel<<<(unsigned)((tot + 255) / 256), 256, 0, (cudaStream_t)stream>>>((const float *)(ws + L.heads), M, cls_score_out, bbox_pred_out);
  CTPN_LAUNCH_CHECK();
  return CTPN_OK;
}

extern "C" int ctpn_net_forward(ctpn_net_t *net, const void *images, int src_is_f32, int B, int H, int W,
                                float *cls_score_out, float *bbox_pred_out, void *workspace, size_t workspace_bytes,
                                void *stream) {
  CTPN_REQUIRE(net && images && cls_score_out && bbox_pred_out && workspace, "ctpn_net_forward: null pointer");
  CTPN_REQUIRE(B > 0 && H >= 16 && W >= 16, "ctpn_net_forward: bad shape B=%d H=%d W=%d", B, H, W);
  return net_forward(net, images, src_is_f32, nullptr, B, H, W, cls_score_out, bbox_pred_out, workspace, workspace_bytes, stream);
}

extern "C" int ctpn_net_forward_ragged(ctpn_net_t *net, const void *images, int src_is_f32, const int *sizes, int B, int H, int W,
                                       float *cls_score_out, float *bbox_pred_out, void *workspace, size_t workspace_bytes,
                                       void *stream) {
  CTPN_REQUIRE(net && images && sizes && cls_score_out && bbox_pred_out && workspace, "ctpn_net_forward_ragged: null pointer");
  CTPN_REQUIRE(B > 0 && H >= 16 && W >= 16, "ctpn_net_forward_ragged: bad shape B=%d H=%d W=%d", B, H, W);
  return net_forward(net, images, src_is_f32, sizes, B, H, W, cls_score_out, bbox_pred_out, workspace, workspace_bytes, stream);
}

extern "C" int ctpn_net_debug_tap(ctpn_net_t *net, const char *name, float *out_f32, size_t capacity, size_t *count,
                                  void *stream) {
  CTPN_REQUIRE(net && name && count, "ctpn_net_debug_tap: null pointer");
  auto it = net->taps.find(name);
  CTPN_REQUIRE(it != net->taps.end(), "ctpn_net_debug_tap: no activation named '%s' (run a forward first)", name);
  const Tap &t = it->second;
  const long long n = t.pixels * t.channels;
  *count = (size_t)n;
  if (!out_f32) return CTPN_OK;
  CTPN_REQUIRE(capacity >= (size_t)n, "ctpn_net_debug_tap: buffer too small (%zu < %lld)", capacity, n);
  const long long stored = t.stack_h ? n / t.stack_h * (t.stack_h + 1) : n;
  if (t.planes && t.q_s > 0.f) {
    f16f8_to_f32_kernel<<<(unsigned)((n + 255) / 256), 256, 0, (cudaStream_t)stream>>>((const __half *)t.ptr, (const uint8_t *)t.ptr + stored * 2, n,
                                                                                       t.channels, t.q_s, t.q_t, t.stack_h, t.stack_w, out_f32);
    CTPN_LAUNCH_CHECK();
  } else if (t.planes) {
    planes_to_f32_kernel<<<(unsigned)((n + 255) / 256), 256, 0, (cudaStream_t)stream>>>((const __nv_bfloat16 *)t.ptr, n, stored, net->planes, t.channels,
                                                                                        t.stack_h, t.stack_w, out_f32);
    CTPN_LAUNCH_CHECK();
  } else {
    CTPN_CUDA(cudaMemcpyAsync(out_f32, t.ptr, (size_t)n * sizeof(float), cudaMemcpyDeviceToDevice, (cudaStream_t)stream));
  }
  return CTPN_OK;
}

#ifdef CTPN_DEBUG
extern "C" int ctpn_net_f16f8_scales(const ctpn_net_t *net, float *s, float *t, float *amax) {
  CTPN_REQUIRE(net && s && t && amax, "ctpn_net_f16f8_scales: null pointer");
  CTPN_REQUIRE(net->f16f8 && net->calibrated, "ctpn_net_f16f8_scales: not a calibrated F16F8 net");
  for (int l = 0; l < 13; ++l) { s[l] = net->act_s[l]; t[l] = net->act_t[l]; amax[l] = net->act_max[l]; }
  return CTPN_OK;
}
#endif
```

text-detection-ctpn_b200/ctpn_b200/_native.py:

```python
import ctypes as C
import os

_HERE = os.path.dirname(os.path.abspath(__file__))
LIB_PATH = os.path.join(_HERE, "libctpn_b200.so")
DEBUG_LIB = os.environ.get("CTPN_B200_LIB", "") == "dbg"
if DEBUG_LIB:
    LIB_PATH = os.path.join(os.path.dirname(os.path.dirname(_HERE)), "tests", "_native", "libctpn_b200_dbg.so")


class CtpnError(RuntimeError):
    pass


ERR_INVALID, ERR_CUDA, ERR_WORKSPACE, ERR_NO_DEVICE = 1, 2, 3, 4


if not os.path.exists(LIB_PATH):
    raise ImportError(
        "libctpn_b200.so is not built (%s). Run `python -c 'import __graft_entry__ as g; g.build()'` "
        "or `make -C text-detection-ctpn_b200/csrc`. There is no CPU fallback." % LIB_PATH)

lib = C.CDLL(LIB_PATH)

_p = C.c_void_p
_i = C.c_int
_f = C.c_float
_z = C.c_size_t

SIGNATURES = {
    "ctpn_version": (_i, []),
    "ctpn_last_error": (C.c_char_p, []),
    "ctpn_device_ok": (_i, [_i]),
    "ctpn_prof_enable": (_i, [_i]),
    "ctpn_prof_report": (_i, [_p, _z, C.POINTER(_z)]),
    "ctpn_crc32c_host": (C.c_uint32, [_p, _z, C.c_uint32]),
    "ctpn_nms_host": (_i, [_p, _p, _p, _i, _i, _f, _i]),
    "ctpn_text_lines_host": (_i, [_p, _p, _i, _i, _i, _i, _p, _p, _i, _p]),
    "ctpn_text_lines_workspace_bytes": (_z, [_i, _i, _i]),
    "ctpn_text_lines": (_i, [_p, _p, _i, _i, _p, _p, _i, _p, _p, _p, _p, _p, _z, _p]),
    "ctpn_text_filter_nms_host": (_i, [_p, _p, _i, _p, _p, _p]),
    "ctpn_text_groups_host": (_i, [_p, _p, _i, _i, _p, _p, _p, _i, _p, _p]),
    "ctpn_bbox_overlaps_host": (_i, [_p, _i, _i, _p, _i, _i, _p]),
    "ctpn_bbox_intersections_host": (_i, [_p, _i, _i, _p, _i, _i, _p]),
    "ctpn_anchor_targets_host": (_i, [_p, _i, _i, _p, _p, _i, _i, _i, _i, C.c_double, C.c_double, _p, _p, _p]),
    "ctpn_resize_out_size": (_i, [_i, _i, C.c_double, C.c_double, _p, _p]),
    "ctpn_resize_linear_u8": (_i, [_p, _i, _i, _i, _i, C.c_double, C.c_double, _p, _i, _i, _p]),
    "ctpn_image_blob_f32": (_i, [_p, _p, _i, _i, _i, C.c_double, C.c_double, _p, _i, _i, _p]),
    "ctpn_resize_linear_u8_ragged": (_i, [_p, _z, _p, _p, _p, _p, _i, _i, _p, _i, _i, _p]),
    "ctpn_image_blob_f32_ragged": (_i, [_p, _z, _p, _p, _p, _p, _p, _i, _p, _i, _i, _p]),
    "ctpn_resize_linear_u8_ragged_rows": (_i, [_p, _z, _p, _p, _p, _p, _z, _p, _p, _p, _i, _i, _p, _i, _i, _p]),
    "ctpn_resize_linear_u8_strided": (_i, [_p, _p, _p, _p, _p, _p, _p, _i, _p, _i, _i, _p]),
    "ctpn_nms_workspace_bytes": (_z, [_i, _i]),
    "ctpn_nms_sorted": (_i, [_p, _p, _i, _i, _f, _i, _p, _p, _p, _z, _p]),
    "ctpn_proposals_workspace_bytes": (_z, [_i, _i, _i, _i]),
    "ctpn_proposals": (_i, [_p, _i, _p, _p, _i, _i, _i, _i, _i, _i, _f, _f, _i, _p, _p, _p, _p, _z, _p]),
    "ctpn_proposals_ragged": (_i, [_p, _i, _p, _p, _p, _i, _i, _i, _i, _i, _i, _f, _f, _i, _p, _p, _p, _p, _z, _p]),
    "ctpn_pack_weights": (_i, [_p, _i, _i, _i, _i, _i, _p, _p]),
    "ctpn_pack_weights_f16f8": (_i, [_p, _i, _i, _i, _i, _f, _f, _p, _p]),
    "ctpn_conv3x3_f16f8": (_i, [_p, _p, _p, _p, _i, _i, _i, _i, _i, _i, _i, _f, _f, _f, _f, _p]),
    "ctpn_conv1_1_tc_f16f8": (_i, [_p, _i, _p, _p, _p, _p, _i, _i, _i, _f, _f, _p]),
    "ctpn_conv1_1_tc": (_i, [_p, _i, _p, _p, _p, _p, _i, _i, _i, _i, _p]),
    "ctpn_conv3x3": (_i, [_p, _p, _p, _p, _i, _i, _i, _i, _i, _i, _i, _i, _p]),
    "ctpn_bilstm_recurrent": (_i, [_p, _p, _p, _p, _i, _i, _i, _p]),
    "ctpn_net_create": (_i, [C.POINTER(_p), _i]),
    "ctpn_net_destroy": (_i, [_p]),
    "ctpn_net_set_option": (_i, [_p, C.c_char_p, _i]),
    "ctpn_net_set_weight": (_i, [_p, C.c_char_p, _p, _z]),
    "ctpn_net_workspace_bytes": (_z, [_p, _i, _i, _i]),
    "ctpn_net_forward": (_i, [_p, _p, _i, _i, _i, _i, _p, _p, _p, _z, _p]),
    "ctpn_net_forward_ragged": (_i, [_p, _p, _i, _p, _i, _i, _i, _p, _p, _p, _z, _p]),
    "ctpn_net_feature_hw": (_i, [_i, _i, C.POINTER(_i), C.POINTER(_i)]),
    "ctpn_net_debug_tap": (_i, [_p, C.c_char_p, _p, _z, C.POINTER(_z), _p]),
}

TESTING_SIGNATURES = {
    "ctpn_conv1_1": (_i, [_p, _i, _p, _p, _p, _p, _i, _i, _i, _i, _p]),
    "ctpn_conv3x3_simt": (_i, [_p, _p, _p, _p, _i, _i, _i, _i, _i, _i, _i, _i, _p]),
    "ctpn_probe_umma_view": (_i, [_p, _p, _i, _i, _i, _i, _p, _p]),
    "ctpn_net_f16f8_scales": (_i, [_p, _p, _p, _p]),
}

for _name, (_res, _args) in list(SIGNATURES.items()) + (list(TESTING_SIGNATURES.items()) if DEBUG_LIB else []):
    _fn = getattr(lib, _name)
    _fn.restype = _res
    _fn.argtypes = _args


def prof_report():
    import json
    need = C.c_size_t()
    check(lib.ctpn_prof_report(None, 0, C.byref(need)), "ctpn_prof_report")
    buf = C.create_string_buffer(need.value)
    check(lib.ctpn_prof_report(buf, need.value, C.byref(need)), "ctpn_prof_report")
    return json.loads(buf.value.decode())


def last_error():
    return lib.ctpn_last_error().decode("utf-8", "replace")


def check(status, what=""):
    if status != 0:
        raise CtpnError("%s failed (status %d): %s" % (what or "ctpn call", status, last_error()))


def ptr(t):
    if t is None:
        return None
    if hasattr(t, "data_ptr"):
        return C.c_void_p(t.data_ptr())
    return C.c_void_p(t.ctypes.data)


def stream_ptr(stream=None):
    import torch
    s = stream if stream is not None else torch.cuda.current_stream()
    return C.c_void_p(s.cuda_stream)
```

Measured before the change: 817.8.

## Fuse conv1_1 into conv1_2 tensor-core kernel, building im2col tiles in shared memory

Result: faster. 835.6 (median of 6 runs) (+2.2%).

```diff
diff --git a/text-detection-ctpn_b200/csrc/common.cuh b/text-detection-ctpn_b200/csrc/common.cuh
--- a/text-detection-ctpn_b200/csrc/common.cuh
+++ b/text-detection-ctpn_b200/csrc/common.cuh
@@ -45,8 +45,11 @@
 int conv1_1_tc_ragged(const void *src, int src_is_f32, const float *lut, const float *w_hwio, const float *bias, void *out_planes,
                       int B, int H, int W, int planes, bool outq, float out_s, float out_t, const int *sizes, void *stream);
 struct QuantScales { float inv_main, inv_cross, out_s, out_t; };
+struct Conv1Input { const void *src; int src_is_f32; const float *lut, *w, *bias; float out_s, out_t; };
 int conv_tc_run(const void *in_planes, const void *w_planes, const float *bias, void *out, int B, int H, int W, int cin,
-                int cout, int taps, int planes, int flags, const QuantScales *q, const int *ext, int ext_shift, void *stream);
+                int cout, int taps, int planes, int flags, const QuantScales *q, const int *ext, int ext_shift, void *stream,
+                const Conv1Input *c1 = nullptr);
+int conv_tc_conv1_fusable(int B, int H, int W, int planes, bool *fusable);
 int bilstm_ragged(const float *xproj, const float *wh_fw, const float *wh_bw, void *out_planes, int R, int W, int planes,
                   const int *sizes, int rows_per_image, void *stream);
 
diff --git a/text-detection-ctpn_b200/csrc/conv1_tc.cu b/text-detection-ctpn_b200/csrc/conv1_tc.cu
--- a/text-detection-ctpn_b200/csrc/conv1_tc.cu
+++ b/text-detection-ctpn_b200/csrc/conv1_tc.cu
@@ -1,6 +1,7 @@
 #include <mutex>
 
 #include "common.cuh"
+#include "conv1_tile.cuh"
 #include "tc_ptx.cuh"
 
 namespace ctpn {
@@ -64,26 +65,7 @@
   }
   if (!p.src_is_f32)
     for (int i = threadIdx.x; i < 768; i += kC1tThreads) lut_s[i] = p.lut[i];
-  for (int i = threadIdx.x; i < 64 * 4; i += kC1tThreads) {
-    const int co = i >> 2, chunk = i & 3;
-    uint32_t pk[3][4];
-#pragma unroll
-    for (int j = 0; j < 4; ++j) {
-      float v[2];
-#pragma unroll
-      for (int e = 0; e < 2; ++e) {
-        const int k = chunk * 8 + j * 2 + e;
-        v[e] = k < 27 ? p.w[k * 64 + co] : (k == 27 ? p.bias[co] : 0.f);
-      }
-      uint32_t t[P];
-      split_planes2<P>(v[0], v[1], t);
-#pragma unroll
-      for (int pl = 0; pl < P; ++pl) pk[pl][j] = t[pl];
-    }
-#pragma unroll
-    for (int pl = 0; pl < P; ++pl)
-      *reinterpret_cast<uint4 *>(bsm + pl * 64 * 128 + co * 128 + ((chunk ^ (co & 7)) << 4)) = make_uint4(pk[pl][0], pk[pl][1], pk[pl][2], pk[pl][3]);
-  }
+  c1_weight_tile<P>(p.w, p.bias, bsm, threadIdx.x, kC1tThreads);
   fence_proxy_async();
   __syncthreads();
   const int tiles_per_img = p.tiles_x * p.tiles_y;
@@ -147,27 +129,9 @@
       mbar_wait(emptyA + 8 * s, ph ^ 1u);
       if (grp == 0) asm volatile("bar.sync 1, 128;" ::: "memory");
       else asm volatile("bar.sync 2, 128;" ::: "memory");
-      uint8_t *arow = base + s * P * kC1tTileBytes + m * 128;
-#pragma unroll
-      for (int chunk = 0; chunk < (C1_DBG(p, 2) ? 0 : 4); ++chunk) {
-        uint32_t pk[3][4];
-#pragma unroll
-        for (int j = 0; j < 4; ++j) {
-          float v[2];
-#pragma unroll
-          for (int e = 0; e < 2; ++e) {
-            const int k = chunk * 8 + j * 2 + e;
-            v[e] = k < 27 ? pt[((k % 3) * 18 + th + k / 9) * 40 + tw + (k / 3) % 3] : (k == 27 ? 1.f : 0.f);
-          }
-          uint32_t t[P];
-          split_planes2<P>(v[0], v[1], t);
-#pragma unroll
-          for (int pl = 0; pl < P; ++pl) pk[pl][j] = t[pl];
-        }
-#pragma unroll
-        for (int pl = 0; pl < P; ++pl)
-          *reinterpret_cast<uint4 *>(arow + pl * kC1tTileBytes + ((chunk ^ (m & 7)) << 4)) = make_uint4(pk[pl][0], pk[pl][1], pk[pl][2], pk[pl][3]);
-      }
+      if (!C1_DBG(p, 2))
+        c1_im2col_row<P>(base + s * P * kC1tTileBytes + m * 128, m, kC1tTileBytes,
+                         [&](int k) { return pt[((k % 3) * 18 + th + k / 9) * 40 + tw + (k / 3) % 3]; });
       fence_proxy_async();
       mbar_arrive(fullA + 8 * s);
     }
@@ -176,7 +140,6 @@
     const int cw = warp - 8, chunk = cw >> 2, quarter = cw & 3;
     const int m = quarter * 32 + lane, th = m >> 3, tw = m & 7;
     const int frow = wg * 64 + (warp & 3) * 16 + (lane >> 2);
-    constexpr uint32_t kHi = gmma_desc_hi(1024);
     const uint32_t b_lo = gmma_desc_lo(b0);
     float accm[32], accc[32];
     uint4 *stage_w = reinterpret_cast<uint4 *>(epi + chunk * 4096 + quarter * 1024);
@@ -202,17 +165,7 @@
       mbar_wait(fullA + 8 * s, ph);
       const uint32_t a_lo = gmma_desc_lo(a0 + s * P * kC1tTileBytes + wg * 64 * 128);
       wgmma_fence();
-#pragma unroll
-      for (int i = 0; i < P; ++i)
-#pragma unroll
-        for (int j = 0; j < P - i; ++j)
-#pragma unroll
-          for (int k = 0; k < 2; ++k) {
-            const uint64_t da = ((uint64_t)kHi << 32) | (a_lo + i * (kC1tTileBytes >> 4) + 2u * k);
-            const uint64_t db = ((uint64_t)kHi << 32) | (b_lo + j * ((64 * 128) >> 4) + 2u * k);
-            if (i + j == 0) wgmma_bf16(accm, da, db, (uint32_t)k);
-            else wgmma_bf16(accc, da, db, (k == 0 && i == 0 && j == 1) ? 0u : 1u);
-          }
+      c1_mmas<P>(accm, accc, a_lo, kC1tTileBytes >> 4, b_lo);
       wgmma_commit();
       wgmma_wait<0>();
       wgmma_fence_regs(accm);
diff --git a/text-detection-ctpn_b200/csrc/conv1_tile.cuh b/text-detection-ctpn_b200/csrc/conv1_tile.cuh
--- /dev/null
+++ b/text-detection-ctpn_b200/csrc/conv1_tile.cuh
@@ -0,0 +1,77 @@
+#pragma once
+
+#include "common.cuh"
+#include "tc_ptx.cuh"
+
+namespace ctpn {
+
+constexpr int kC1RowBytes = 128;
+constexpr int kC1WeightBytes = 64 * kC1RowBytes;
+
+template <int P>
+__device__ __forceinline__ void c1_weight_tile(const float *w, const float *bias, uint8_t *bsm, int tid, int nthreads) {
+  for (int i = tid; i < 64 * 4; i += nthreads) {
+    const int co = i >> 2, chunk = i & 3;
+    uint32_t pk[3][4];
+#pragma unroll
+    for (int j = 0; j < 4; ++j) {
+      float v[2];
+#pragma unroll
+      for (int e = 0; e < 2; ++e) {
+        const int k = chunk * 8 + j * 2 + e;
+        v[e] = k < 27 ? w[k * 64 + co] : (k == 27 ? bias[co] : 0.f);
+      }
+      uint32_t t[P];
+      split_planes2<P>(v[0], v[1], t);
+#pragma unroll
+      for (int pl = 0; pl < P; ++pl) pk[pl][j] = t[pl];
+    }
+#pragma unroll
+    for (int pl = 0; pl < P; ++pl)
+      *reinterpret_cast<uint4 *>(bsm + pl * kC1WeightBytes + co * kC1RowBytes + ((chunk ^ (co & 7)) << 4)) =
+          make_uint4(pk[pl][0], pk[pl][1], pk[pl][2], pk[pl][3]);
+  }
+}
+
+template <int P, typename Tap>
+__device__ __forceinline__ void c1_im2col_row(uint8_t *arow, int row, int plane_bytes, Tap tap) {
+#pragma unroll
+  for (int chunk = 0; chunk < 4; ++chunk) {
+    uint32_t pk[3][4];
+#pragma unroll
+    for (int j = 0; j < 4; ++j) {
+      float v[2];
+#pragma unroll
+      for (int e = 0; e < 2; ++e) {
+        const int k = chunk * 8 + j * 2 + e;
+        v[e] = k < 27 ? tap(k) : (k == 27 ? 1.f : 0.f);
+      }
+      uint32_t t[P];
+      split_planes2<P>(v[0], v[1], t);
+#pragma unroll
+      for (int pl = 0; pl < P; ++pl) pk[pl][j] = t[pl];
+    }
+#pragma unroll
+    for (int pl = 0; pl < P; ++pl)
+      *reinterpret_cast<uint4 *>(arow + pl * plane_bytes + ((chunk ^ (row & 7)) << 4)) = make_uint4(pk[pl][0], pk[pl][1], pk[pl][2], pk[pl][3]);
+  }
+}
+
+template <int P>
+__device__ __forceinline__ void c1_mmas(float (&accm)[32], float (&accc)[32], uint32_t a_lo, uint32_t a_plane16, uint32_t b_lo) {
+  using namespace ptx;
+  constexpr uint32_t kHi = gmma_desc_hi(1024);
+#pragma unroll
+  for (int i = 0; i < P; ++i)
+#pragma unroll
+    for (int j = 0; j < P - i; ++j)
+#pragma unroll
+      for (int k = 0; k < 2; ++k) {
+        const uint64_t da = ((uint64_t)kHi << 32) | (a_lo + i * a_plane16 + 2u * k);
+        const uint64_t db = ((uint64_t)kHi << 32) | (b_lo + j * (kC1WeightBytes >> 4) + 2u * k);
+        if (i + j == 0) wgmma_bf16(accm, da, db, (uint32_t)k);
+        else wgmma_bf16(accc, da, db, (k == 0 && i == 0 && j == 1) ? 0u : 1u);
+      }
+}
+
+}
diff --git a/text-detection-ctpn_b200/csrc/conv_tc.cu b/text-detection-ctpn_b200/csrc/conv_tc.cu
--- a/text-detection-ctpn_b200/csrc/conv_tc.cu
+++ b/text-detection-ctpn_b200/csrc/conv_tc.cu
@@ -5,6 +5,7 @@
 #include <unordered_map>
 
 #include "common.cuh"
+#include "conv1_tile.cuh"
 #include "tc_ptx.cuh"
 #include "tma_host.cuh"
 
@@ -38,6 +39,10 @@
   int ext_shift, ext_n;
   double work;
   int promote_every;
+  const void *c1_src;
+  const float *c1_lut, *c1_w, *c1_bias;
+  int c1_f32;
+  float c1_s, c1_t, c1_rs;
 };
 
 template <int BN, int PR> constexpr bool kEpiWarpgroup = !PR && BN <= 128;
@@ -46,6 +51,11 @@
 constexpr int kCtrlBytes = 8 * (4 * kMaxStages) + 16;
 constexpr int kEpiBytes = 2 * 128 * 32 * 4;
 constexpr int kXposeBytes = 4 * 512;
+constexpr int kC1Region = 13312;
+constexpr int kC1Im2col = 128 * kC1RowBytes;
+constexpr int kC1Patch = 3 * 20 * 12;
+template <int P> constexpr int kC1Bytes = 2 * P * kC1Im2col + P * kC1WeightBytes + (((kC1Patch + 768) * 4 + 1023) & ~1023);
+constexpr int kC1Builders = 96;
 
 struct EpiPixel {
   bool ok, live;
@@ -202,7 +212,7 @@
   }
 }
 
-template <int BN, int P, int TAPS, int MC, int F8, int PR = 0>
+template <int BN, int P, int TAPS, int MC, int F8, int PR = 0, int C1 = 0>
 __global__ void __launch_bounds__(kTcThreads<BN, PR>, 1)
 conv_tc_kernel(const __grid_constant__ CUtensorMap tmap_a, const __grid_constant__ CUtensorMap tmap_b,
                const ConvTcParams p) {
@@ -211,11 +221,16 @@
   constexpr bool EW = kEpiWarpgroup<BN, PR>;
   static_assert(!F8 || P == 2, "F16F8 uses two stage slots per operand");
   static_assert(!PR || (P == 3 && !F8), "promotion is built for three bf16 planes");
+  static_assert(!C1 || (TAPS == 9 && BN == 64 && !MC && !PR && P <= 2), "conv1_1 is fused into the single-CTA conv1_2 only");
   extern __shared__ uint8_t smem_raw[];
   const uint32_t raw = smem_u32(smem_raw);
   const uint32_t ring_a = (raw + 1023u) & ~1023u;
-  const uint32_t a_stage = (uint32_t)P * p.patch_bytes, b_stage = (uint32_t)P * kBBytes;
-  const uint32_t ring_b = ring_a + (uint32_t)p.stages_a * a_stage;
+  const uint32_t a_stage = C1 ? 2u * P * kC1Region : (uint32_t)P * p.patch_bytes, b_stage = (uint32_t)P * kBBytes;
+  const uint32_t c1_base = ring_a + (uint32_t)p.stages_a * a_stage;
+  const uint32_t c1_w = c1_base + 2u * P * kC1Im2col;
+  float *c1_patch = reinterpret_cast<float *>(smem_raw + (c1_w - raw) + P * kC1WeightBytes);
+  float *c1_lut = c1_patch + kC1Patch;
+  const uint32_t ring_b = c1_base + (C1 ? (uint32_t)kC1Bytes<P> : 0u);
   float *epi = reinterpret_cast<float *>(smem_raw + (ring_b - raw) + (size_t)p.stages_b * b_stage);
   uint4 *xpose = reinterpret_cast<uint4 *>(reinterpret_cast<uint8_t *>(epi) + kEpiBytes);
   uint8_t *ctrl = reinterpret_cast<uint8_t *>(epi) + kEpiBytes + (EW ? kXposeBytes : 0);
@@ -228,14 +243,23 @@
     prefetch_tmap(&tmap_a);
     prefetch_tmap(&tmap_b);
     for (int s = 0; s < kMaxStages; ++s) {
-      mbar_init(fullA + 8 * s, 1);
-      mbar_init(emptyA + 8 * s, 2);
+      mbar_init(fullA + 8 * s, C1 ? kC1Builders : 1);
+      mbar_init(emptyA + 8 * s, C1 ? 1 : 2);
       mbar_init(fullB + 8 * s, 1);
       mbar_init(emptyB + 8 * s, MC ? 4 : 2);
     }
     mbar_init(epiF, 256);
     mbar_init(epiE, 128);
     fence_mbar_init();
+  }
+  if constexpr (C1) {
+    c1_weight_tile<P>(p.c1_w, p.c1_bias, smem_raw + (c1_w - raw), threadIdx.x, blockDim.x);
+    if (!p.c1_f32)
+      for (int i = threadIdx.x; i < 768; i += blockDim.x) c1_lut[i] = p.c1_lut[i];
+    for (int i = threadIdx.x; i < 2 * P * 28 * 8; i += blockDim.x)
+      *reinterpret_cast<uint4 *>(smem_raw + (c1_base - raw) + (i / 224) * kC1Im2col + (100 + (i % 224) / 8) * 128 + (i % 8) * 16) =
+          make_uint4(0u, 0u, 0u, 0u);
+    fence_proxy_async();
   }
   __syncthreads();
   if (MC) cluster_sync_all();
@@ -252,9 +276,65 @@
   constexpr int halo = TAPS == 9 ? 1 : 0;
 
   if (warp < 4) {
-    if (EW) regs_dealloc<24>();
-    else regs_dealloc<40>();
-    if (warp == 1) {
+    if (!C1) {
+      if (EW) regs_dealloc<24>();
+      else regs_dealloc<40>();
+    }
+    if (C1 && warp >= 1) {
+      const int bt = threadIdx.x - 32;
+      uint32_t ph = 0;
+      for (int u = u_begin; u < p.total_units; u += u_step) {
+        int mt, nt;
+        unit_tile(u, mt, nt);
+        const int b = mt / tiles_per_img, r = mt % tiles_per_img;
+        const int y0 = (r / p.tiles_x) * p.TH, x0 = (r % p.tiles_x) * p.TW;
+        int eh = p.H, ew = p.W;
+        if (p.ext) {
+          eh = min(eh, __ldg(p.ext + 2 * b));
+          ew = min(ew, __ldg(p.ext + 2 * b + 1));
+        }
+        uint32_t raw3[3][3];
+        unsigned valid = 0;
+#pragma unroll
+        for (int it = 0; it < 3; ++it) {
+          const int i = bt + it * kC1Builders, gy = y0 - 2 + i / 12, gx = x0 - 2 + i % 12;
+          if (i < 240 && gy >= 0 && gy < eh && gx >= 0 && gx < ew) {
+            const size_t off = (((size_t)b * p.H + gy) * p.W + gx) * 3;
+            if (p.c1_f32) {
+              const float *q = reinterpret_cast<const float *>(p.c1_src) + off;
+              raw3[it][0] = __float_as_uint(q[0]); raw3[it][1] = __float_as_uint(q[1]); raw3[it][2] = __float_as_uint(q[2]);
+            } else {
+              const uint8_t *q = reinterpret_cast<const uint8_t *>(p.c1_src) + off;
+              raw3[it][0] = q[0]; raw3[it][1] = q[1]; raw3[it][2] = q[2];
+            }
+            valid |= 1u << it;
+          }
+        }
+        named_sync(4, kC1Builders);
+#pragma unroll
+        for (int it = 0; it < 3; ++it) {
+          const int i = bt + it * kC1Builders;
+          if (i < 240) {
+#pragma unroll
+            for (int c = 0; c < 3; ++c)
+              c1_patch[c * 240 + i] = !((valid >> it) & 1u) ? 0.f : p.c1_f32 ? __uint_as_float(raw3[it][c]) : c1_lut[raw3[it][c] * 3 + c];
+          }
+        }
+        named_sync(4, kC1Builders);
+#pragma unroll 1
+        for (int w = 0; w < 2; ++w) {
+          mbar_wait(emptyA + 8 * w, ph ^ 1u);
+          for (int rr = bt; rr < 100; rr += kC1Builders) {
+            const float *pt = c1_patch + (8 * w + rr / 10) * 12 + rr % 10;
+            c1_im2col_row<P>(smem_raw + (c1_base - raw) + w * P * kC1Im2col + rr * 128, rr, kC1Im2col,
+                             [&](int k) { return pt[(k % 3) * 240 + (k / 9) * 12 + (k / 3) % 3]; });
+          }
+          fence_proxy_async();
+          mbar_arrive(fullA + 8 * w);
+        }
+        ph ^= 1u;
+      }
+    } else if (warp == 1 && !C1) {
       int s = 0;
       uint32_t ph = 0;
       for (int u = u_begin; u < p.total_units; u += u_step) {
@@ -306,7 +386,7 @@
       }
     }
   } else if (EW && warp >= 12) {
-    regs_alloc<152>();
+    if (!C1) regs_alloc<152>();
     const int m = (warp & 3) * 32 + lane;
     uint4 *stage_w = xpose + (warp & 3) * 32;
     uint32_t eph = 0;
@@ -336,7 +416,8 @@
       }
     }
   } else {
-    if (EW) regs_alloc<168>();
+    if (C1) {}
+    else if (EW) regs_alloc<168>();
     else regs_alloc<232>();
     const int wg = (warp >> 2) - 1;
     const bool leader = (threadIdx.x & 127) == 0;
@@ -348,11 +429,12 @@
 #else
     constexpr int pe = 1;
 #endif
-    constexpr uint32_t kPatch16 = (TAPS == 9 ? 23552u : 16384u) >> 4;
+    constexpr uint32_t kPatch16 = (C1 ? (uint32_t)kC1Region : TAPS == 9 ? 23552u : 16384u) >> 4;
     constexpr uint32_t kB16 = (uint32_t)kBBytes >> 4;
     constexpr uint32_t kHiB = gmma_desc_hi(1024);
     const uint32_t hi_a = gmma_desc_hi((uint32_t)p.group_stride_bytes);
-    const uint32_t wg_off = (uint32_t)wg * 8u * (uint32_t)p.group_stride_bytes;
+    const uint32_t wg_off = C1 ? (uint32_t)wg * P * kC1Region : (uint32_t)wg * 8u * (uint32_t)p.group_stride_bytes;
+    uint32_t c1ph = 0;
     int sa = 0, sb = 0, prev_b = -1, prev_a = -1;
     uint32_t pha = 0, phb = 0, eph = 0;
     const int frow = wg * 64 + (warp & 3) * 16 + (lane >> 2);
@@ -380,6 +462,76 @@
       }
     };
     for (int u = u_begin; u < p.total_units; u += u_step) {
+      if constexpr (C1) {
+        int mt, nt;
+        unit_tile(u, mt, nt);
+        const int b = mt / tiles_per_img, r = mt % tiles_per_img;
+        const int y0 = (r / p.tiles_x) * p.TH - 1, x0 = (r % p.tiles_x) * p.TW - 1;
+        int eh = p.H, ew = p.W;
+        if (p.ext) {
+          eh = min(eh, __ldg(p.ext + 2 * b));
+          ew = min(ew, __ldg(p.ext + 2 * b + 1));
+        }
+        uint8_t *region = smem_raw + (ring_a - raw) + wg_off;
+        named_sync(2 + wg, 128);
+        mbar_wait(fullA + 8 * wg, c1ph);
+        c1ph ^= 1u;
+#pragma unroll 1
+        for (int blk = 0; blk < 2; ++blk) {
+          wgmma_fence();
+          c1_mmas<P>(accm, accc, gmma_desc_lo(c1_base + wg * P * kC1Im2col + blk * 64 * 128), kC1Im2col >> 4, gmma_desc_lo(c1_w));
+          wgmma_commit();
+          wgmma_wait<0>();
+          wgmma_fence_regs(accm);
+          if (P > 1) wgmma_fence_regs(accc);
+          if (blk == 1 && leader) mbar_arrive(emptyA + 8 * wg);
+#pragma unroll
+          for (int h = 0; h < 2; ++h) {
+            const int rr = blk * 64 + (warp & 3) * 16 + (lane >> 2) + 8 * h;
+            if (rr < 100) {
+              const int y = y0 + 8 * wg + rr / 10, x = x0 + rr % 10;
+              const bool live = y >= 0 && y < eh && x >= 0 && x < ew;
+              uint8_t *row = region + rr * 128;
+              const int sw = rr & 7, q4 = 4 * (lane & 3);
+              float v[16];
+#pragma unroll
+              for (int i8 = 0; i8 < 8; ++i8) {
+#pragma unroll
+                for (int e = 0; e < 2; ++e) {
+                  float t = accm[4 * i8 + 2 * h + e];
+                  if (P > 1) t = t + accc[4 * i8 + 2 * h + e];
+                  if (!live) t = 0.f;
+                  v[2 * i8 + e] = fmaxf(t, 0.f);
+                }
+              }
+              if (F8) {
+#pragma unroll
+                for (int i8 = 0; i8 < 8; i8 += 2) {
+                  uint32_t h01, h23, qv, qr;
+                  f16f8_quad(v[2 * i8], v[2 * i8 + 1], v[2 * i8 + 2], v[2 * i8 + 3], p.c1_s, p.c1_t, p.c1_rs, h01, h23, qv, qr);
+                  *reinterpret_cast<uint32_t *>(row + ((i8 ^ sw) << 4) + q4) = h01;
+                  *reinterpret_cast<uint32_t *>(row + (((i8 + 1) ^ sw) << 4) + q4) = h23;
+                  uint8_t *row1 = row + kC1Region;
+                  *reinterpret_cast<uint16_t *>(row1 + (((i8 >> 1) ^ sw) << 4) + q4 / 2) = (uint16_t)qv;
+                  *reinterpret_cast<uint16_t *>(row1 + (((i8 >> 1) ^ sw) << 4) + 8 + q4 / 2) = (uint16_t)(qv >> 16);
+                  *reinterpret_cast<uint16_t *>(row1 + (((4 + (i8 >> 1)) ^ sw) << 4) + q4 / 2) = (uint16_t)qr;
+                  *reinterpret_cast<uint16_t *>(row1 + (((4 + (i8 >> 1)) ^ sw) << 4) + 8 + q4 / 2) = (uint16_t)(qr >> 16);
+                }
+              } else {
+#pragma unroll
+                for (int i8 = 0; i8 < 8; ++i8) {
+                  uint32_t t[P];
+                  split_planes2<P>(v[2 * i8], v[2 * i8 + 1], t);
+#pragma unroll
+                  for (int pl = 0; pl < P; ++pl) *reinterpret_cast<uint32_t *>(row + pl * kC1Region + ((i8 ^ sw) << 4) + q4) = t[pl];
+                }
+              }
+            }
+          }
+        }
+        fence_proxy_async();
+        named_sync(2 + wg, 128);
+      }
       if (PR) {
 #pragma unroll
         for (int i = 0; i < R; ++i) accs[i] = 0.f;
@@ -390,7 +542,7 @@
           release(prev_b, prev_a);
           prev_b = prev_a = -1;
         }
-        mbar_wait(fullA + 8 * sa, pha);
+        if (!C1) mbar_wait(fullA + 8 * sa, pha);
         const uint32_t a_lo = gmma_desc_lo(ring_a + sa * a_stage + wg_off);
 #pragma unroll
         for (int tap = 0; tap < TAPS; ++tap) {
@@ -450,7 +602,7 @@
           wgmma_wait<1>();
           if (prev_b >= 0) release(prev_b, prev_a);
           prev_b = sb;
-          prev_a = tap == TAPS - 1 ? sa : -1;
+          prev_a = tap == TAPS - 1 && !C1 ? sa : -1;
           if (PR && ((step + 1) % pe == 0 || step == kblocks * TAPS - 1)) {
             wgmma_fence_regs(accm);
 #pragma unroll
@@ -582,23 +734,25 @@
   return CTPN_OK;
 }
 
-template <int BN, int P, int TAPS, int MC, int F8 = 0, int PR = 0>
+template <int BN, int P, int TAPS, int MC, int F8 = 0, int PR = 0, int C1 = 0>
 static int launch_bn(int dev, const CUtensorMap &ta, const CUtensorMap &tb, ConvTcParams &p, cudaStream_t st) {
-  const size_t a_stage = (size_t)p.planes * p.patch_bytes, b_stage = (size_t)p.planes * BN * 128;
+  const size_t a_stage = C1 ? (size_t)2 * P * kC1Region : (size_t)p.planes * p.patch_bytes, b_stage = (size_t)p.planes * BN * 128;
   const size_t epi_bytes = kEpiBytes + (kEpiWarpgroup<BN, PR> ? kXposeBytes : 0);
-  const size_t budget = 227 * 1024 - 1024 - kCtrlBytes - epi_bytes;
+  const size_t c1_bytes = C1 ? kC1Bytes<P> : 0;
+  const size_t budget = 227 * 1024 - 1024 - kCtrlBytes - epi_bytes - c1_bytes;
   int sa = (2 * a_stage + 2 * b_stage <= budget) ? 2 : 1;
   if (p.taps == 1) sa = (int)std::min<size_t>(4, std::max<size_t>(1, (budget / 2) / a_stage));
+  if (C1) sa = 1;
   CTPN_REQUIRE(sa * a_stage + 2 * b_stage <= budget, "conv_tc: pipeline stages (%zu + 2 x %zu B) do not fit in shared memory", a_stage, b_stage);
   int sb = (int)((budget - sa * a_stage) / b_stage);
   if (sb > kMaxStages) sb = kMaxStages;
-  if (tuning().stages_a > 0) sa = std::max(1, std::min(sa, tuning().stages_a));
+  if (tuning().stages_a > 0 && !C1) sa = std::max(1, std::min(sa, tuning().stages_a));
   if (tuning().stages_b > 0) sb = std::max(2, std::min(sb, tuning().stages_b));
   p.stages_a = sa;
   p.stages_b = sb;
-  const size_t smem = 1024 + sa * a_stage + sb * b_stage + epi_bytes + kCtrlBytes;
+  const size_t smem = 1024 + sa * a_stage + c1_bytes + sb * b_stage + epi_bytes + kCtrlBytes;
   CTPN_REQUIRE(smem <= 227 * 1024, "conv_tc: %zu bytes of shared memory", smem);
-  auto kernel = conv_tc_kernel<BN, P, TAPS, MC, F8, PR>;
+  auto kernel = conv_tc_kernel<BN, P, TAPS, MC, F8, PR, C1>;
   static bool attr_set[kMaxDevices];
   static int max_clusters[kMaxDevices];
   cudaLaunchConfig_t cfg = {};
@@ -634,13 +788,50 @@
   return CTPN_OK;
 }
 
+static void pick_tiles(int dev, int B, int H, int W, int cout, int taps, int planes, bool promote, int &BN, bool &mc) {
+  BN = tuning().bn > 0 ? tuning().bn : (planes == 1 ? 256 : 128);
+  if (!(BN == 64 || BN == 128 || BN == 256)) BN = 256;
+  if (planes > 1 && BN > 128) BN = 128;
+  while (BN > cout || cout % BN) BN >>= 1;
+  const long long tiles_x = taps == 9 ? ceil_div(W, 8) : ceil_div(W, 128), tiles_y = taps == 9 ? ceil_div(H, 16) : H;
+  const long long m_tiles = (long long)B * tiles_x * tiles_y;
+  constexpr long long kMcMaxTilesPerSm = 16;
+  mc = taps == 9 && tuning().mcast != 0 && m_tiles >= 2 &&
+       (promote || m_tiles * (cout / BN) < kMcMaxTilesPerSm * g_sms[dev]);
+  if (promote && taps == 9 && !mc && BN > 64) BN = 64;
+}
+
+static int device_sms(int &dev, const char *what) {
+  CTPN_CUDA(cudaGetDevice(&dev));
+  CTPN_REQUIRE(dev >= 0 && dev < kMaxDevices, "%s: device index %d not supported", what, dev);
+  std::lock_guard<std::mutex> lock(g_mu);
+  if (g_sms[dev] == 0) CTPN_CUDA(cudaDeviceGetAttribute(&g_sms[dev], cudaDevAttrMultiProcessorCount, dev));
+  return CTPN_OK;
+}
+
+int conv_tc_conv1_fusable(int B, int H, int W, int planes, bool *fusable) {
+  int dev = 0, BN = 0, rc;
+  bool mc = false;
+  if ((rc = device_sms(dev, "conv_tc_conv1_fusable"))) return rc;
+  pick_tiles(dev, B, H, W, 64, 9, planes, false, BN, mc);
+  *fusable = planes <= 2 && !mc;
+  return CTPN_OK;
+}
+
 int conv_tc_run(const void *in_planes, const void *w_planes, const float *bias, void *out, int B, int H, int W, int cin,
-                int cout, int taps, int planes, int flags, const QuantScales *q, const int *ext, int ext_shift, void *stream) {
+                int cout, int taps, int planes, int flags, const QuantScales *q, const int *ext, int ext_shift, void *stream,
+                const Conv1Input *c1) {
   const bool f8 = q != nullptr, promote = (flags & CTPN_F_PROMOTE) != 0;
   CTPN_REQUIRE(f8 || !(flags & CTPN_F_OUT_BF16X2), "ctpn_conv3x3: CTPN_F_OUT_BF16X2 is a flag of ctpn_conv3x3_f16f8");
   CTPN_REQUIRE(!(promote && f8), "ctpn_conv3x3_f16f8: CTPN_F_PROMOTE is a flag of ctpn_conv3x3 with planes = 3");
   CTPN_REQUIRE(!promote || planes == 3, "ctpn_conv3x3: CTPN_F_PROMOTE needs planes = 3 (got %d)", planes);
-  CTPN_REQUIRE(in_planes && w_planes && bias && out, "ctpn_conv3x3: null pointer");
+  CTPN_REQUIRE((in_planes || c1) && w_planes && bias && out, "ctpn_conv3x3: null pointer");
+  if (c1) {
+    CTPN_REQUIRE(c1->src && c1->w && c1->bias && (c1->src_is_f32 || c1->lut), "conv1_1 + conv1_2: null pointer");
+    CTPN_REQUIRE(taps == 9 && cin == 64 && cout == 64 && planes <= 2 && !promote &&
+                 (flags & ~(CTPN_F_RELU | CTPN_F_POOL)) == 0 && (flags & CTPN_F_POOL),
+                 "conv1_1 + conv1_2: needs a pooled 64 -> 64 3x3 layer on one or two planes");
+  }
   CTPN_REQUIRE(taps == 9 || taps == 1, "ctpn_conv3x3: taps must be 9 or 1 (got %d)", taps);
   CTPN_REQUIRE(planes >= 1 && planes <= 3, "ctpn_conv3x3: planes must be 1..3 (got %d)", planes);
   CTPN_REQUIRE(cin % 64 == 0 && cin >= 64, "ctpn_conv3x3: Cin must be a multiple of 64 (got %d)", cin);
@@ -658,12 +849,7 @@
     B = 1;
   }
   int dev = 0, rc;
-  CTPN_CUDA(cudaGetDevice(&dev));
-  CTPN_REQUIRE(dev >= 0 && dev < kMaxDevices, "ctpn_conv3x3: device index %d not supported", dev);
-  {
-    std::lock_guard<std::mutex> lock(g_mu);
-    if (g_sms[dev] == 0) CTPN_CUDA(cudaDeviceGetAttribute(&g_sms[dev], cudaDevAttrMultiProcessorCount, dev));
-  }
+  if ((rc = device_sms(dev, "ctpn_conv3x3"))) return rc;
 
   ConvTcParams p;
   memset(&p, 0, sizeof(p));
@@ -705,15 +891,20 @@
   p.debug = tuning().debug;
   p.promote_every = tuning().promote;
 
-  int BN = tuning().bn > 0 ? tuning().bn : (planes == 1 ? 256 : 128);
-  if (!(BN == 64 || BN == 128 || BN == 256)) BN = 256;
-  if (planes > 1 && BN > 128) BN = 128;
-  while (BN > cout || cout % BN) BN >>= 1;
+  int BN;
+  bool mc;
+  pick_tiles(dev, B, H, W, cout, taps, planes, promote, BN, mc);
   const long long m_tiles = (long long)B * p.tiles_x * p.tiles_y;
-  constexpr long long kMcMaxTilesPerSm = 16;
-  const bool mc = taps == 9 && tuning().mcast != 0 && m_tiles >= 2 &&
-                  (promote || m_tiles * (cout / BN) < kMcMaxTilesPerSm * g_sms[dev]);
-  if (promote && taps == 9 && !mc && BN > 64) BN = 64;
+  if (c1) {
+    CTPN_REQUIRE(!mc, "conv1_1 + conv1_2: the map is small enough for the multicast kernel, which has no fused conv1_1");
+    BN = 64;
+    p.c1_src = c1->src; p.c1_lut = c1->lut; p.c1_w = c1->w; p.c1_bias = c1->bias; p.c1_f32 = c1->src_is_f32;
+    p.c1_s = p.c1_t = p.c1_rs = 1.f;
+    if (f8) {
+      CTPN_REQUIRE(c1->out_s > 0.f && c1->out_t > 0.f, "conv1_1 + conv1_2: scales must be positive");
+      p.c1_s = c1->out_s; p.c1_t = c1->out_t; p.c1_rs = kResidualGain * c1->out_t / c1->out_s;
+    }
+  }
   p.tiles_n = cout / BN;
   const long long total = m_tiles * p.tiles_n;
   CTPN_REQUIRE(total < (1ll << 31), "ctpn_conv3x3: too many tiles");
@@ -722,7 +913,7 @@
   p.total_units = mc ? (int)((m_tiles + 1) / 2) * p.tiles_n : p.total_tiles;
 
   CUtensorMap ta, tb;
-  {
+  if (!c1) {
     const int halo = taps == 9 ? 1 : 0;
     cuuint64_t dims[4] = {(cuuint64_t)cin, (cuuint64_t)W, (cuuint64_t)H, (cuuint64_t)planes * B};
     cuuint64_t strides[3] = {(cuuint64_t)cin * 2, (cuuint64_t)W * cin * 2, (cuuint64_t)H * W * cin * 2};
@@ -735,7 +926,13 @@
     cuuint32_t box[2] = {64, (cuuint32_t)(mc ? BN / 2 : BN)};
     if ((rc = cached_tmap(dev, &tb, w_planes, 2, dims, strides, box))) return rc;
   }
+  if (c1) ta = tb;
   cudaStream_t st = (cudaStream_t)stream;
+  if (c1) {
+    if (f8) return launch_bn<64, 2, 9, 0, 1, 0, 1>(dev, ta, tb, p, st);
+    if (planes == 2) return launch_bn<64, 2, 9, 0, 0, 0, 1>(dev, ta, tb, p, st);
+    return launch_bn<64, 1, 9, 0, 0, 0, 1>(dev, ta, tb, p, st);
+  }
 #define CTPN_TC_CASE(BN_, P_, T_) \
   if (BN == BN_ && planes == P_ && taps == T_) return launch_bn<BN_, P_, T_, 0>(dev, ta, tb, p, st)
 #define CTPN_TC_CASE_MC(BN_, P_) \
@@ -789,3 +986,24 @@
   const QuantScales q{inv_main, inv_cross, out_s, out_t};
   return conv_tc_run(in_planes, w_planes, bias, out, B, H, W, cin, cout, taps, 2, flags, &q, nullptr, 0, stream);
 }
+
+#ifdef CTPN_DEBUG
+#include "testing/ctpn_b200_testing.h"
+
+extern "C" int ctpn_conv1_12_tc(const void *src, int src_is_f32, const float *lut, const float *w11, const float *b11,
+                                const void *w12_planes, const float *b12, void *mid, void *out, const int *sizes, int B, int H,
+                                int W, int planes, int f16f8, const float *scales, int fuse, void *stream) {
+  CTPN_REQUIRE(scales, "ctpn_conv1_12_tc: null scales");
+  CTPN_REQUIRE(!f16f8 || planes == 2, "ctpn_conv1_12_tc: F16F8 carries two planes");
+  const QuantScales q{scales[2], scales[3], scales[4], scales[5]};
+  const float s1 = f16f8 ? scales[0] : 1.f, t1 = f16f8 ? scales[1] : 1.f;
+  const int flags = CTPN_F_RELU | CTPN_F_POOL;
+  if (fuse) {
+    const Conv1Input c1{src, src_is_f32, lut, w11, b11, s1, t1};
+    return conv_tc_run(nullptr, w12_planes, b12, out, B, H, W, 64, 64, 9, planes, flags, f16f8 ? &q : nullptr, sizes, 1, stream, &c1);
+  }
+  int rc = conv1_1_tc_ragged(src, src_is_f32, lut, w11, b11, mid, B, H, W, planes, f16f8 != 0, s1, t1, sizes, stream);
+  if (rc) return rc;
+  return conv_tc_run(mid, w12_planes, b12, out, B, H, W, 64, 64, 9, planes, flags, f16f8 ? &q : nullptr, sizes, 1, stream);
+}
+#endif
diff --git a/text-detection-ctpn_b200/csrc/net.cu b/text-detection-ctpn_b200/csrc/net.cu
--- a/text-detection-ctpn_b200/csrc/net.cu
+++ b/text-detection-ctpn_b200/csrc/net.cu
@@ -38,6 +38,7 @@
   float w_s[14] = {0}, w_t[14] = {0}, act_s[14] = {0}, act_t[14] = {0}, act_max[14] = {0};
   unsigned *absmax_dev = nullptr;
   int conv_simt = 0, keep = 0;
+  bool fuse_conv1 = true;
   std::map<std::string, std::vector<float>> host;
   bool dirty = true;
   std::vector<void *> owned;
@@ -292,7 +293,7 @@
 }
 
 static int run_conv(ctpn_net *n, const NetLayout &L, int l, const void *images, int src_is_f32, const int *sizes, int B,
-                    char *ws, float out_s, float out_t, void *stream) {
+                    char *ws, float out_s, float out_t, void *stream, bool fused = false) {
   const ConvSpec &s = kConvs[l];
   const ConvLayer &c = L.conv[l];
   if (!n->f16f8 || (c.flags & CTPN_F_OUT_BF16X2)) out_s = out_t = 1.f;
@@ -309,8 +310,9 @@
                              out_t, sizes, stream);
   QuantScales q{};
   if (n->f16f8) q = {1.f / (n->act_s[l - 1] * n->w_s[l]), 1.f / (kResidualGain * n->act_t[l - 1] * n->w_t[l]), out_s, out_t};
-  return conv_tc_run(ws + c.in, n->conv_w[l], n->conv_b[l], ws + c.out, B, c.h, c.w, s.cin, s.cout, 9, n->planes, c.flags,
-                     n->f16f8 ? &q : nullptr, sizes, c.shift, stream);
+  const Conv1Input c1{images, src_is_f32, n->lut, n->c11_w, n->c11_b, n->f16f8 ? n->act_s[0] : 1.f, n->f16f8 ? n->act_t[0] : 1.f};
+  return conv_tc_run(fused ? nullptr : ws + c.in, n->conv_w[l], n->conv_b[l], ws + c.out, B, c.h, c.w, s.cin, s.cout, 9, n->planes,
+                     c.flags, n->f16f8 ? &q : nullptr, sizes, c.shift, stream, fused ? &c1 : nullptr);
 }
 
 static int calibrate_f16f8(ctpn_net *n, const void *images, int src_is_f32, const int *sizes, int B, const NetLayout &L, char *ws,
@@ -374,6 +376,7 @@
   CTPN_REQUIRE(net && key, "ctpn_net_set_option: null pointer");
   if (!strcmp(key, "keep_activations")) net->keep = value != 0;
   else if (!strcmp(key, "recalibrate")) net->calibrated = false;
+  else if (!strcmp(key, "fuse_conv1")) net->fuse_conv1 = value != 0;
 #ifdef CTPN_DEBUG
   else if (!strcmp(key, "conv_simt")) {
     CTPN_REQUIRE(!value || !net->f16f8, "ctpn_net_set_option: the SIMT reference kernels read bf16 planes, not F16F8");
@@ -419,10 +422,12 @@
   const int P = net->planes;
   net->taps.clear();
   if (net->f16f8 && !net->calibrated && (rc = calibrate_f16f8(net, images, src_is_f32, sizes, B, L, ws, stream))) return rc;
-  for (int l = 0; l < 14; ++l) {
+  bool fuse = net->fuse_conv1 && P <= 2 && !net->promote && !net->keep && !net->conv_simt;
+  if (fuse && (rc = conv_tc_conv1_fusable(B, H, W, P, &fuse))) return rc;
+  for (int l = fuse ? 1 : 0; l < 14; ++l) {
     const ConvSpec &s = kConvs[l];
     const ConvLayer &c = L.conv[l];
-    if ((rc = run_conv(net, L, l, images, src_is_f32, sizes, B, ws, net->act_s[l], net->act_t[l], stream))) return rc;
+    if ((rc = run_conv(net, L, l, images, src_is_f32, sizes, B, ws, net->act_s[l], net->act_t[l], stream, fuse && l == 1))) return rc;
     const bool q = net->f16f8 && !(c.flags & CTPN_F_OUT_BF16X2);
     net->taps[s.pool ? std::string(s.name) + "+pool" : std::string(s.name)] =
         Tap{ws + c.out, (long long)B * c.ho * c.wo, s.cout, true, q ? net->act_s[l] : 0.f, q ? net->act_t[l] : 0.f,
diff --git a/text-detection-ctpn_b200/ctpn_b200/_native.py b/text-detection-ctpn_b200/ctpn_b200/_native.py
--- a/text-detection-ctpn_b200/ctpn_b200/_native.py
+++ b/text-detection-ctpn_b200/ctpn_b200/_native.py
@@ -78,6 +78,7 @@
     "ctpn_conv3x3_simt": (_i, [_p, _p, _p, _p, _i, _i, _i, _i, _i, _i, _i, _i, _p]),
     "ctpn_probe_umma_view": (_i, [_p, _p, _i, _i, _i, _i, _p, _p]),
     "ctpn_net_f16f8_scales": (_i, [_p, _p, _p, _p]),
+    "ctpn_conv1_12_tc": (_i, [_p, _i, _p, _p, _p, _p, _p, _p, _p, _p, _i, _i, _i, _i, _i, _p, _i, _p]),
 }
 
 for _name, (_res, _args) in list(SIGNATURES.items()) + (list(TESTING_SIGNATURES.items()) if DEBUG_LIB else []):
```
